# george-tyler-315-incline/ggml-neon-opt

Measured on AMD Instinct MI355X. Metric: tg128 tok/s + Q4_K GEMV achieved-HBM-GB/s, TinyLlama-1.1B Q4_K_M @1 GPU, higher is better.
Workload: dtype q4_K/q6_K x q8_K (u4/u6*i8 dot4 -> i32, f32 combine); 1 GPU; tinyllama-1.1b Q4_K_M tg2221: full decode graph, token i at position i of a fresh f16 KV cache; parallelism=replicas x1, hipgraph=True

## Files before the change

ggml-neon-opt_amd/csrc/kq_api.hip:

```cpp
#include <algorithm>
#include <stdio.h>
#include <stdlib.h>
#include <string.h>

#include <atomic>
#include <mutex>
#include <string>
#include <vector>

#include <hip/hip_ext.h>

#include "kq_common.h"
#include "kq_internal.h"

namespace kq {

template <int NCOL, bool FUSEDQ, bool DEBUG, int TMASK>
__global__ void kq_gemv(const GemvArgs a);
__global__ void kq_quantize_q8K(const float *x, int64_t x_stride, uint8_t *y, int nb, int64_t nblocks);
template <int TMASK, bool FUSEDQ, int PRO>
__global__ void kq_rows(const RowsArgs a);
template <int TMASK, bool FUSEDQ, int PRO>
__global__ void kq_rows_dyn(const RowsArgs a);
template <bool AM>
__global__ void kq_quantize_q8L(const float *x, int64_t x_stride, uint8_t *y, int nb, int64_t nblocks);
template <int TYPE, int RT, int CW>
__global__ void kq_mmq(const MmqArgs a);
template <int RT, int CW>
__global__ void kq_mmq_mixed(const MmqArgs a);
__global__ void kq_stream_ceiling(const uint8_t *buf, int64_t per_wave, int waves_total, uint32_t *sink);
__global__ void kq_quantize_f16img(const float *x, int64_t x_stride, uint8_t *img, uint8_t *bs, int nb, int64_t nblocks);
template <int TYPE, int NW>
__global__ void kq_mmf(const MmfArgs a);
__global__ void kq_mmf_reduce(const float *slab, int n_split, int m_cols, int n_rows, int slab_rows, float *y,
                              int64_t y_col_stride, const float *res, int64_t res_col_stride);

namespace {

constexpr int kMaxDevices = 64;
std::mutex g_dev_mu;
std::atomic<int> g_dev_state[kMaxDevices];
int g_dev_cus[kMaxDevices] = {0};

int current_device() {
    int dev = 0;
    if (hipGetDevice(&dev) != hipSuccess || dev < 0 || dev >= kMaxDevices) return -1;
    return dev;
}

void probe_device(int dev) {
    int n = 0;
    if (hipGetDeviceCount(&n) != hipSuccess || n <= 0 || dev >= n) {
        g_dev_state[dev].store(-1);
        return;
    }
    hipDeviceProp_t prop;
    if (hipGetDeviceProperties(&prop, dev) != hipSuccess) {
        g_dev_state[dev].store(-1);
        return;
    }
    if (strncmp(prop.gcnArchName, "gfx950", 6) != 0) {
        fprintf(stderr, "ggml_mi355x: device %d is %s, this library is built for gfx950 only\n", dev,
                prop.gcnArchName);
        g_dev_state[dev].store(-1);
        return;
    }
    g_dev_cus[dev] = prop.multiProcessorCount > 0 ? prop.multiProcessorCount : 256;
    g_dev_state[dev].store(1, std::memory_order_release);
}

template <int NCOL, bool FUSEDQ, bool DEBUG>
gemv_fn pick_tm(int tmask) {
    switch (tmask) {
        case 1: return kq_gemv<NCOL, FUSEDQ, DEBUG, 1>;
        case 4: return kq_gemv<NCOL, FUSEDQ, DEBUG, 4>;
        default: return kq_gemv<NCOL, FUSEDQ, DEBUG, 7>;
    }
}

gemv_fn pick_gemv(int ncol, bool fusedq, bool debug, int tmask) {
    if (debug) return pick_tm<1, false, true>(tmask);
    if (fusedq) return pick_tm<1, true, false>(tmask);
    switch (ncol) {
        case 1: return pick_tm<1, false, false>(tmask);
        case 2: return pick_tm<2, false, false>(tmask);
        case 4: return pick_tm<4, false, false>(tmask);
        default: return pick_tm<8, false, false>(tmask);
    }
}

int type_bit(int type) { return type == Q4_K ? 1 : type == Q5_K ? 2 : type == Q6_K ? 4 : 0; }

constexpr size_t kMaxLds = 160 * 1024;
constexpr size_t kTargetLds = 80 * 1024;
constexpr int64_t kFusedQMaxNb = 32;
constexpr int64_t kRowsFusedMaxNb = ROWS_QPASS * 4 * ROWS_WAVES;
constexpr double kRowsSmallBytes = 5e6;
std::atomic<int> g_rows_waves{0};

struct KnobDef {
    const char *name;
    double def;
};
const KnobDef kKnobs[KNOB_COUNT] = {
    {"GEMV_DIAG", 0},  {"GEMV_RING", 0},     {"GEMV_PRE0", 1},       {"GEMV_PF", 0},
    {"GEMV_XMODE", 0}, {"GEMV_SMALL_MB", kRowsSmallBytes / 1e6},      {"GEMV_WPC", 0},
    {"GEMV_SMALL_WG", 0}, {"GEMV_FQMAX", (double)kRowsFusedMaxNb},   {"MMF_WAVES", 0},
    {"MMF_ORDER", 0},  {"ATTN_DIAG", 0},     {"LOOPBACK_NOCOPY", 0}, {"ATTN_OPROJ", 1},
    {"AO_NRB", 0},     {"GEMV_DYN", 8},    {"GEMV_DYN_P", 0},      {"GEMV_DYN_STEPS", 16},
};
std::atomic<double> g_knob[KNOB_COUNT];
std::atomic<bool> g_knob_set[KNOB_COUNT];
std::atomic<uint32_t> g_knob_gen{0};


uint64_t *g_stamps = nullptr;
int64_t g_stamps_cap = 0;

struct OccKey {
    int dev;
    const void *fn;
    size_t lds;
};
int resident_wgs(const void *fn, size_t lds) {
    static std::mutex mu;
    static std::vector<std::pair<OccKey, int>> cache;
    const int dev = current_device();
    std::lock_guard<std::mutex> lk(mu);
    for (auto &e : cache)
        if (e.first.dev == dev && e.first.fn == fn && e.first.lds == lds) return e.second;
    int n = 0;
    if (lds > 64 * 1024) hipFuncSetAttribute(fn, hipFuncAttributeMaxDynamicSharedMemorySize, (int)kMaxLds);
    if (hipOccupancyMaxActiveBlocksPerMultiprocessor(&n, fn, WG_THREADS, lds) != hipSuccess || n <= 0) n = 1;
    if (n > 8) n = 8;
    cache.push_back({{dev, fn, lds}, n});
    return n;
}

}

double knob(Knob k) { return g_knob_set[k].load(std::memory_order_relaxed) ? g_knob[k].load() : kKnobs[k].def; }
uint32_t knob_generation() { return g_knob_gen.load(); }

struct TimedLaunch {
    std::string kernel;
    double bytes;
    hipEvent_t start, stop;
};
std::mutex g_tmu;
bool g_timing = false;
std::vector<TimedLaunch> g_tlog;
std::vector<std::pair<hipEvent_t, hipEvent_t>> g_tpool;
size_t g_tpool_used = 0;

bool capturing(hipStream_t s) {
    hipStreamCaptureStatus st = hipStreamCaptureStatusNone;
    if (hipStreamIsCapturing(s, &st) != hipSuccess) return false;
    return st != hipStreamCaptureStatusNone;
}

bool timing_slot(hipStream_t s, hipEvent_t &a, hipEvent_t &b) {
    std::lock_guard<std::mutex> lk(g_tmu);
    if (!g_timing || capturing(s)) return false;
    if (g_tpool_used == g_tpool.size()) {
        hipEvent_t e0, e1;
        if (hipEventCreate(&e0) != hipSuccess) return false;
        if (hipEventCreate(&e1) != hipSuccess) {
            hipEventDestroy(e0);
            return false;
        }
        g_tpool.push_back({e0, e1});
    }
    a = g_tpool[g_tpool_used].first;
    b = g_tpool[g_tpool_used].second;
    ++g_tpool_used;
    return true;
// ... 200 lines not shown
            if (((uintptr_t)d[i].w & 3u) != 0) return MI355X_E_INVAL;
            if (d[i].row_stride != (size_t)(nb * bb)) return MI355X_E_UNSUPPORTED;
            if (d[i].type != Q6_K && ((uintptr_t)d[i].w & 15u)) return MI355X_E_UNSUPPORTED;
        }
        bytes_total += (double)d[i].n_rows * bb;
        tmask |= type_bit(d[i].type);
    }
    if (tmask != 1 && tmask != 2 && tmask != 4) tmask = 7;
    pl.tmask = tmask;
    pl.fusedq = fusedq;
    pl.fn = pick_rows(tmask, fusedq, ROWS_PRO_NONE);
    a.n_desc = n_desc;
    a.nb = (int)nb;
    for (int i = 0; i < n_desc; ++i) {
        a.type[i] = d[i].type;
        a.w[i] = (const uint8_t *)d[i].w;
        a.y[i] = d[i].y;
        a.n_rows[i] = (int)d[i].n_rows;
    }
    {
        a.pf = (int)knob(KNOB_GEMV_PF);
        a.xmode = (int)knob(KNOB_GEMV_XMODE) & 7;
        a.diag = (int)knob(KNOB_GEMV_DIAG);
        const int pre = (int)knob(KNOB_GEMV_PRE0);
        a.pre0 = pre < 0 ? 0 : pre > 3 ? 3 : pre;
    }
    a.stamps = g_stamps;
    a.stamps_cap = g_stamps_cap;
    const double small_bytes = knob(KNOB_GEMV_SMALL_MB) * 1e6;
    if (waves_per_cu <= 0) {
        const int fixed = g_rows_waves.load();
        const int want = fixed > 0 ? fixed : bytes_total * nb < small_bytes ? ROWS_WAVES_SMALL : ROWS_WAVES;
        waves_per_cu = !fusedq || nb <= ROWS_QPASS * 4 * want ? want : ROWS_WAVES;
    }
    if (waves_per_cu > ROWS_WAVES) return MI355X_E_INVAL;
    pl.nwv = waves_per_cu;
    const int wpc_env = (int)knob(KNOB_GEMV_WPC);
    if (wpc_env > 0 && wpc_env < waves_per_cu) waves_per_cu = wpc_env;
    const int small_wg_env = (int)knob(KNOB_GEMV_SMALL_WG);
    int64_t n_wg = num_cus();
    if (small_wg_env > 0 && bytes_total * nb < small_bytes && small_wg_env < n_wg) n_wg = small_wg_env;
    const int64_t cap = n_wg * waves_per_cu;
    int64_t wv[MI355X_MAX_FUSED] = {0, 0, 0, 0};
    int64_t waves = 0;
    for (int i = 0; i < n_desc; ++i) {
        if (d[i].n_rows == 0) continue;
        const double share = (double)d[i].n_rows * block_bytes(d[i].type) / bytes_total;
        int64_t w = (int64_t)(share * (double)cap);
        const int64_t min_rows = (ROWS_SB + nb - 1) / nb;
        const int64_t wmax = (d[i].n_rows + min_rows - 1) / min_rows;
        if (w > wmax) w = wmax;
        if (w < 1) w = 1;
        wv[i] = w;
        waves += w;
    }
    while (waves > cap) {
        int big = 0;
        for (int i = 1; i < n_desc; ++i)
            if (wv[i] > wv[big]) big = i;
        --wv[big];
        --waves;
    }
    int64_t rpw = 0;
    waves = 0;
    for (int i = 0; i < n_desc; ++i) {
        a.wave_prefix[i] = (int)waves;
        if (wv[i] > 0) {
            a.rbase[i] = (int)(d[i].n_rows / wv[i]);
            a.rrem[i] = (int)(d[i].n_rows % wv[i]);
            const int64_t r = a.rbase[i] + (a.rrem[i] ? 1 : 0);
            rpw = r > rpw ? r : rpw;
        }
        waves += wv[i];
    }
    for (int i = n_desc; i <= MI355X_MAX_FUSED; ++i) a.wave_prefix[i] = (int)waves;
    a.waves_total = (int)waves;
    a.prio_bytes = 0;
    for (int i = 0; i < n_desc; ++i)
        if (wv[i] > 0) {
            const int64_t b = (int64_t)(a.rbase[i] + (a.rrem[i] ? 1 : 0)) * nb * block_bytes(d[i].type);
            a.prio_bytes = b > a.prio_bytes ? b : a.prio_bytes;
        }
    if (rpw > 0x7fffffff / 64) return MI355X_E_UNSUPPORTED;
    a.rpw = (int)(rpw > 0 ? rpw : 1);
    int g16 = ROWS_SB;
    while (nb % g16) g16 >>= 1;
    const int u = ROWS_SB / g16;
    int bR_full = (int)(ROWS_RECS / nb) / u * u;
    if (bR_full < u) bR_full = u;
    a.bR = a.rpw <= bR_full ? a.rpw : bR_full;
    const RowsLayout L = rows_layout((int)nb, tmask, a.bR, a.rpw, pl.nwv);
    if ((size_t)L.total > kMaxLds) return MI355X_E_UNSUPPORTED;
    pl.lds = (size_t)L.total;
    const int64_t grid = waves < n_wg ? waves : n_wg;
    pl.grid = dim3((unsigned)(grid > 0 ? grid : 1), 1, 1);
    pl.dyn = false;
    const double dyn_min = knob(KNOB_GEMV_DYN);
    const bool force = g_impl.load() == MI355X_GEMV_DYN;
    bool same_rows = true;
    for (int i = 1; i < n_desc; ++i) same_rows = same_rows && d[i].n_rows == d[0].n_rows;
    if (tmask != 7 && same_rows && (force || dyn_min > 0)) {
        int ush = 0;
        while ((int64_t)(1 << ush) * nb < ROWS_SB) ++ush;
        const double steps_per_wave = (double)n_desc * d[0].n_rows * nb / ROWS_SB / n_wg / pl.nwv;
        if ((int64_t)(1 << ush) * nb == ROWS_SB && steps_per_wave >= 16) ++ush;
        const int U = 1 << ush;
        const int Tu = (int)((U * nb + ROWS_SB - 1) / ROWS_SB);
        const int D = rows_depth(tmask == 1 ? Q4_K : tmask == 2 ? Q5_K : Q6_K);
        const int64_t flat = (int64_t)n_desc * ((d[0].n_rows + n_wg - 1) / n_wg);
        const int64_t rows = (int64_t)n_desc * d[0].n_rows;
        int bRd = (int)(ROWS_RECS / nb) / U * U;
        if (bRd < U) bRd = U;
        const double per_wave = (double)rows / (double)n_wg / U / pl.nwv;
        const bool auto_ok = per_wave >= dyn_min && steps_per_wave >= knob(KNOB_GEMV_DYN_STEPS);
        const RowsDynLayout DL = rows_dyn_layout((int)nb, tmask, bRd, (int)flat, pl.nwv);
        if ((force || auto_ok) && rows > 0 && (size_t)DL.total <= kMaxLds && flat < 0x7fffffff / 64) {
            pl.dyn = true;
            a.dyn_u = U;
            a.dyn_ush = ush;
            a.rbase[0] = (int)(d[0].n_rows / n_wg);
            a.rrem[0] = (int)(d[0].n_rows % n_wg);
            a.dyn_p = (D + Tu - 1) / Tu;
            const int p_knob = (int)knob(KNOB_GEMV_DYN_P);
            if (p_knob > 0) a.dyn_p = p_knob;
            a.bR = bRd;
            a.rpw = (int)flat;
            pl.lds = (size_t)DL.total;
            pl.grid = dim3((unsigned)n_wg, 1, 1);
            pl.fn = pick_rows(tmask, fusedq, ROWS_PRO_NONE, true);
        }
    }
    return MI355X_OK;
}

std::string rows_name(const RowsPlan &pl) {
    return std::string(pl.dyn ? "kq::kq_rows_dyn<" : "kq::kq_rows<") + std::to_string(pl.tmask) + ", " + (pl.fusedq ? "true" : "false") + ", " +
           std::to_string(pl.a.pro) + ">";
}

double rows_bytes(const RowsArgs &a, bool fusedq) {
    double w = 0, y = 0;
    for (int i = 0; i < a.n_desc; ++i) {
        const double rows = (double)a.n_rows[i];
        w += rows * a.nb * block_bytes(a.type[i]);
        y += rows * 4.0;
    }
    return w + y + (fusedq ? (double)a.nb * QK * 4.0 : (double)a.nb * Q8L_STRIDE);
}

int launch_rows(const RowsPlan &pl, hipStream_t stream) {
    const RowsArgs &a = pl.a;
    if (a.waves_total == 0) return MI355X_OK;
    allow_lds((const void *)pl.fn, pl.lds);
    hipEvent_t e0, e1;
    if (timing_slot(stream, e0, e1)) {
        hipExtLaunchKernelGGL(pl.fn, pl.grid, dim3(pl.nwv * 64), (uint32_t)pl.lds, stream, e0, e1, 0, a);
        timing_log(rows_name(pl), rows_bytes(a, pl.fusedq), e0, e1);
    } else {
        hipLaunchKernelGGL(pl.fn, pl.grid, dim3(pl.nwv * 64), pl.lds, stream, a);
    }
    const hipError_t e = hipGetLastError();
    return e == hipSuccess ? MI355X_OK : (int)e;
}

int launch_quantize_q8L(const float *x, int64_t x_stride_floats, void *y, int64_t k, int64_t nrows,
                        hipStream_t stream, bool mmq) {
    const auto kern = mmq ? kq_quantize_q8L<true> : kq_quantize_q8L<false>;
    const int64_t nb = k / QK;
    const int64_t nblocks = nb * nrows;
    if (nblocks == 0) return MI355X_OK;
    const int64_t wgs = (nblocks + 15) / 16;
    hipEvent_t e0, e1;
    if (timing_slot(stream, e0, e1)) {
        hipExtLaunchKernelGGL(kern, dim3((unsigned)wgs), dim3(WG_THREADS), 0, stream, e0, e1, 0, x,
                              x_stride_floats, (uint8_t *)y, (int)nb, nblocks);
        timing_log("kq::kq_quantize_q8L", (double)nblocks * (QK * 4.0 + Q8L_STRIDE), e0, e1);
    } else {
        hipLaunchKernelGGL(kern, dim3((unsigned)wgs), dim3(WG_THREADS), 0, stream, x, x_stride_floats,
                           (uint8_t *)y, (int)nb, nblocks);
    }
    const hipError_t e = hipGetLastError();
    return e == hipSuccess ? MI355X_OK : (int)e;
}

constexpr int64_t kMmqMinCols = 16;

std::atomic<int> g_mmq_impl{MI355X_MMQ_AUTO};
int mmq_impl() { return g_mmq_impl.load(); }

struct MmqShape {
    int rt, cw;
};
MmqShape mmq_shape(int type, int64_t rows, int64_t M) {
    const int impl = mmq_impl();
    if (impl == MI355X_MMQ_TILE128) return {128, 1};
    if (impl == MI355X_MMQ_TILE128W) return {128, 2};
    if (impl == MI355X_MMQ_TILE64W) return {64, 2};
    if (impl == MI355X_MMQ_TILE64) return {64, 1};
    if (impl == MI355X_MMQ_TILE128X) return {128, type == Q6_K ? 2 : 4};
    if (impl == MI355X_MMQ_TILE192) return type == Q6_K ? MmqShape{128, 1} : MmqShape{192, 1};
    const int64_t rt128 = (rows + 127) / 128;
    const int64_t g128x128 = rt128 * ((M + 127) / 128), g128x64 = rt128 * ((M + 63) / 64);
    if (type != Q6_K && g128x128 >= 160 && g128x128 < 384 && g128x64 >= 512) return {128, 1};
    if (g128x128 >= 160) return {128, 2};
    if (type == Q6_K && ((rows + 63) / 64) * ((M + 127) / 128) >= 192) return {64, 2};
    if (type != Q6_K && rt128 * ((M + 63) / 64) >= 256) return {128, 1};
    return {64, 1};
}
const void *mmq_fn(int type, bool mixed, MmqShape sh) {
#define KQ_MMQ_PICK(RT, CW)                                                      \
    return mixed          ? (const void *)kq_mmq_mixed<RT, CW>                 \
         : type == Q5_K ? (const void *)kq_mmq<Q5_K, RT, CW>                   \
         : type == Q6_K ? (const void *)kq_mmq<Q6_K, RT, CW>                   \
                        : (const void *)kq_mmq<Q4_K, RT, CW>;
    if (sh.rt == 192 && !mixed && type != Q6_K)
        return type == Q5_K ? (const void *)kq_mmq<Q5_K, 192, 1> : (const void *)kq_mmq<Q4_K, 192, 1>;
    if (sh.rt == 128 && sh.cw == 4 && !mixed && type != Q6_K)
        return type == Q5_K ? (const void *)kq_mmq<Q5_K, 128, 4> : (const void *)kq_mmq<Q4_K, 128, 4>;
    if (sh.rt == 128 && sh.cw == 2) KQ_MMQ_PICK(128, 2)
    if (sh.rt == 64 && sh.cw == 2) KQ_MMQ_PICK(64, 2)
    if (sh.rt == 128) KQ_MMQ_PICK(128, 1)
    KQ_MMQ_PICK(64, 1)
#undef KQ_MMQ_PICK
}
size_t mmq_lds(int type, MmqShape sh) {
    return (size_t)mmq_nbuf(type, sh.rt, sh.cw) * (size_t)mmq_buf_bytes(type, sh.rt, sh.cw) + 16 + MMQ_PF_LDS;
}

int launch_mmq(int type, const void *w, int64_t K, int64_t N, size_t row_stride, const uint8_t *xq, int64_t M,
               float *y, int64_t y_col_stride, hipStream_t stream, const float *res, int64_t res_col_stride) {
    MmqArgs a;
    memset(&a, 0, sizeof(a));
    a.n_mat = 1;
    a.res = res;
    a.res_col_stride = res_col_stride;
    a.w = (const uint8_t *)w;
    a.row_stride = (int64_t)row_stride;
    a.n_rows = (int)N;
    a.xq = xq;
    a.nb = (int)(K / QK);
    a.xq_col_stride = (int64_t)a.nb * Q8L_STRIDE;
    a.m_cols = (int)M;
    a.y = y;
    a.y_col_stride = y_col_stride;
    const MmqShape sh = mmq_shape(type, N, M);
    const void *fn = mmq_fn(type, false, sh);
    const size_t lds = mmq_lds(type, sh);
    const int cols = mmq_cols(sh.cw);
    dim3 grid((unsigned)((M + cols - 1) / cols), (unsigned)((N + sh.rt - 1) / sh.rt), 1);
    dim3 block((unsigned)(64 * mmq_waves(sh.rt, sh.cw)));
    std::string name = std::string("kq::kq_mmq<") + std::to_string(type) + ">";
    allow_lds(fn, lds);
    hipEvent_t e0, e1;
    const bool timed = timing_slot(stream, e0, e1);
    void *args[] = {&a};
    hipError_t e;
    if (timed) {
        e = hipExtLaunchKernel(fn, grid, block, args, lds, stream, e0, e1, 0);
        timing_log(name, (double)N * a.nb * block_bytes(type) + (double)M * a.nb * Q8L_STRIDE + (double)M * N * 4.0,
                   e0, e1);
    } else {
        e = hipLaunchKernel(fn, grid, block, args, lds, stream);
    }
    if (e != hipSuccess) return (int)e;
    e = hipGetLastError();
    return e == hipSuccess ? MI355X_OK : (int)e;
}

std::atomic<int> g_prefill{MI355X_PREFILL_EXACT};
int prefill_precision() { return g_prefill.load(); }

int mmf_nw(int64_t K) {
    const int v = (int)knob(KNOB_MMF_WAVES);
    return v == 4 || v == 8 ? v : K >= 8192 ? 8 : 4;
}
struct MmfPlan {
    int nw, n_ct, n_rt, n_split, nbs;
};
MmfPlan mmf_plan_nw(int64_t N, int64_t M, int64_t nb, int nw) {
    MmfPlan p;
    p.nw = nw;
    p.n_ct = (int)((M + MMF_COLS - 1) / MMF_COLS);
    p.n_rt = (int)((N + 32 * nw - 1) / (32 * nw));
    int s = 1;
    while ((int64_t)p.n_ct * p.n_rt * s < 256 && nb >= 8 * s) s *= 2;
    p.nbs = (int)((nb + s - 1) / s);
    p.n_split = (int)((nb + p.nbs - 1) / p.nbs);
    return p;
}
size_t al256(size_t v) { return (v + 255) & ~(size_t)255; }
size_t mmf_workspace(int64_t N, int64_t M, int64_t nb) {
    size_t w = al256((size_t)M * nb * MMF_IMG) + al256((size_t)M * nb * MMF_BSB), slab = 0;
    for (int nw = 4; nw <= 8; nw += 4) {
        const MmfPlan p = mmf_plan_nw(N, M, nb, nw);
        const size_t sb = p.n_split > 1 ? al256((size_t)p.n_split * M * N * 4) : 0;
        slab = sb > slab ? sb : slab;
    }
    return w + slab;
}
bool mmf_prefers(int type, int64_t N, int64_t K) {
    return prefill_precision() == MI355X_PREFILL_F16_ALL || type != Q4_K || N * K >= ((int64_t)32 << 20);
}
bool mmf_applies(int type, const void *w, int64_t N, size_t row_stride, int64_t M, int64_t K) {
    if (prefill_precision() < MI355X_PREFILL_F16) return false;
    if (!rows_enabled() || M < kMmqMinCols || N <= 0) return false;
    if (type != Q4_K && type != Q5_K && type != Q6_K) return false;
    if (N >= (1ll << 31) || M >= (1ll << 31)) return false;
    if (!mmf_prefers(type, N, K)) return false;
    if (type == Q6_K) return true;
    return ((uintptr_t)w & 15u) == 0 && (row_stride & 15u) == 0;
}

// ... 717 lines not shown
```

ggml-neon-opt_amd/csrc/kq_common.h:

```cpp
#pragma once

#include <hip/hip_runtime.h>
#include <stdint.h>

#include "ggml_mi355x.h"

namespace kq {

constexpr int QK = 256;
constexpr int WAVE = 64;
constexpr int WG_THREADS = 256;
constexpr int WAVES_PER_WG = WG_THREADS / WAVE;
constexpr int LANES_PER_BLOCK = 8;
constexpr int BLOCKS_PER_STEP = WAVE / LANES_PER_BLOCK;
constexpr int ACT_QS_STRIDE = 272;
constexpr int MAX_NCOL = 8;

constexpr int Q4_K = MI355X_TYPE_Q4_K;
constexpr int Q5_K = MI355X_TYPE_Q5_K;
constexpr int Q6_K = MI355X_TYPE_Q6_K;

__host__ __device__ constexpr int block_bytes(int type) {
    return type == Q4_K ? 144 : type == Q5_K ? 176 : type == Q6_K ? 210 : 0;
}

struct GemvArgs {
    int n_desc;
    int nb;
    int R;
    int m_total;
    int tasks_total;
    int out_per_wg;
    int diag;
    int ring;
    int ring_override;
    int task_prefix[MI355X_MAX_FUSED + 1];
    int type[MI355X_MAX_FUSED];
    int n_rows[MI355X_MAX_FUSED];
    const uint8_t *w[MI355X_MAX_FUSED];
    int64_t row_stride[MI355X_MAX_FUSED];
    float *y[MI355X_MAX_FUSED];
    int64_t y_col_stride[MI355X_MAX_FUSED];
    const float *x;
    int64_t x_col_stride;
    const uint8_t *xq;
    int64_t xq_col_stride;
    int32_t *dbg;
    uint64_t *stamps;
    int64_t stamps_cap;
};

struct LdsLayout {
    int ring, act, act_per_wave, act_col, recs, outs, spw, total;
};

__host__ __device__ inline LdsLayout lds_layout(int ncol, int nb, int out_per_wg, bool fusedq, int slot, int D) {
    LdsLayout L;
    L.spw = (nb + WAVES_PER_WG - 1) / WAVES_PER_WG;
    L.ring = 0;
    L.act = WAVES_PER_WG * D * slot;
    L.act_col = (L.spw * 292 + 16 + 15) & ~15;
    L.act_per_wave = fusedq ? L.spw * 1024 : ncol * L.act_col;
    L.recs = L.act + WAVES_PER_WG * L.act_per_wave;
    L.outs = L.recs + 2 * (WAVES_PER_WG - 1) * ncol * 8 * L.spw * 16;
    L.total = L.outs + out_per_wg * 4;
    return L;
}

#ifndef KQ_ROWS_WAVES
#define KQ_ROWS_WAVES 12
#endif
constexpr int ROWS_WAVES = KQ_ROWS_WAVES;
#ifndef KQ_ROWS_WAVES_SMALL
#define KQ_ROWS_WAVES_SMALL 6
#endif
constexpr int ROWS_WAVES_SMALL = KQ_ROWS_WAVES_SMALL;
constexpr int ROWS_QPASS = 3;
#ifndef KQ_ROWS_PF
#define KQ_ROWS_PF 2
#endif
constexpr int ROWS_PF = KQ_ROWS_PF;

struct RowsArgs {
    int n_desc;
    int nb;
    int rpw;
    int waves_total;
    int pre0;
    int pf;
    int bR;
    int xmode;
    int diag;
    int wave_prefix[MI355X_MAX_FUSED + 1];
    int rbase[MI355X_MAX_FUSED];
    int rrem[MI355X_MAX_FUSED];
    int type[MI355X_MAX_FUSED];
    const uint8_t *w[MI355X_MAX_FUSED];
    float *y[MI355X_MAX_FUSED];
    const float *x;
    const uint8_t *xq;
    uint64_t *stamps;
    int64_t stamps_cap;
    int pro;
    float eps;
    const float *x2;
    const float *res[MI355X_MAX_FUSED];
    int n_rows[MI355X_MAX_FUSED];
    int epi, epi_n, epi_wave_off;
    float *epi_y;
    int64_t prio_bytes;
    int dyn_u, dyn_p, dyn_ush;
};
constexpr int ROWS_PRO_NONE = 0, ROWS_PRO_NORM = 1, ROWS_PRO_SWIGLU = 2;
constexpr int ROWS_X_ROT = 1, ROWS_X_BAR = 2, ROWS_X_PIPE = 4;

constexpr int ROWS_SB = 16;
#ifndef KQ_MMQ_PF
#define KQ_MMQ_PF 0
#endif
constexpr int MMQ_PF_LDS = KQ_MMQ_PF ? 1024 : 0;
constexpr int Q8L_STRIDE = 304;
#ifndef KQ_MMQ_NBUF
#define KQ_MMQ_NBUF 2
#endif
__host__ __device__ constexpr int mmq_cgroups(int cw) { return cw == 4 ? 1 : 2; }
__host__ __device__ constexpr int mmq_cols(int cw) { return 32 * cw * mmq_cgroups(cw); }
__host__ __device__ constexpr int mmq_waves(int rt, int cw) { return rt / 32 * mmq_cgroups(cw); }
#ifndef KQ_MMQ_Q6_STRIDE
#define KQ_MMQ_Q6_STRIDE 240
#endif
static_assert(KQ_MMQ_Q6_STRIDE % 16 == 0 && KQ_MMQ_Q6_STRIDE >= 224, "whole granules");
__host__ __device__ constexpr int mmq_buf_bytes(int type, int rt, int cw) {
    return mmq_cols(cw) * Q8L_STRIDE + rt * (type == Q6_K ? KQ_MMQ_Q6_STRIDE : block_bytes(type));
}
__host__ __device__ constexpr int mmq_nbuf(int type, int rt, int cw) {
    return KQ_MMQ_NBUF == 1 ? 1 : KQ_MMQ_NBUF >= 3 && ((rt == 128 && cw == 1) || (rt == 64 && cw == 2)) &&
                   3 * mmq_buf_bytes(type, rt, cw) + 16 + MMQ_PF_LDS <= 160 * 1024
               ? 3
               : 2;
}
constexpr int ROWS_RECS = 64;
__host__ __device__ constexpr int rows_gran(int type) { return block_bytes(type) + 1; }
__host__ __device__ constexpr int rows_slot(int type) { return 16 * rows_gran(type); }
__host__ __device__ constexpr int rows_ni(int type) { return (rows_gran(type) + 63) / 64; }
#ifndef KQ_ROWS_DQ4
#define KQ_ROWS_DQ4 3
#endif
#ifndef KQ_ROWS_DQ6
#define KQ_ROWS_DQ6 2
#endif
__host__ __device__ constexpr int rows_depth(int type) {
    return type == Q4_K ? KQ_ROWS_DQ4 : type == Q5_K ? 3 : KQ_ROWS_DQ6;
}
__host__ __device__ constexpr int rows_ring_bytes(int type) { return rows_depth(type) * rows_slot(type); }
__host__ __device__ constexpr int cmax(int a, int b) { return a > b ? a : b; }
__host__ __device__ constexpr int rows_ring(int tmask) {
    return 16 + cmax((tmask & 1) ? rows_ring_bytes(Q4_K) : 0,
                     cmax((tmask & 2) ? rows_ring_bytes(Q5_K) : 0, (tmask & 4) ? rows_ring_bytes(Q6_K) : 0));
}

struct RowsLayout {
    int act, ring, ring_stride, recs, recs_stride, outs, outs_stride, sums, total;
};
__host__ __device__ inline RowsLayout rows_layout(int nb, int tmask, int bR, int rpw, int nwv) {
    RowsLayout L;
    L.act = 0;
    L.ring = nb * Q8L_STRIDE;
    L.ring_stride = rows_ring(tmask);
    L.recs = L.ring + nwv * L.ring_stride;
    L.recs_stride = bR * nb * 16;
    L.outs = L.recs + nwv * L.recs_stride;
    L.outs_stride = (rpw * 4 + 15) & ~15;
    L.sums = L.outs + nwv * L.outs_stride;
    L.total = L.sums + nb * 8;
    return L;
}

struct RowsDynLayout {
    int act, ring, ring_stride, recs, recs_stride, outs, sums, cnt, total;
};
__host__ __device__ inline RowsDynLayout rows_dyn_layout(int nb, int tmask, int bR, int flat_rows, int nwv) {
    RowsDynLayout L;
    L.act = 0;
    L.ring = nb * Q8L_STRIDE;
    L.ring_stride = rows_ring(tmask);
    L.recs = L.ring + nwv * L.ring_stride;
    L.recs_stride = bR * nb * 16;
    L.outs = L.recs + nwv * L.recs_stride;
    L.sums = L.outs + ((flat_rows * 4 + 15) & ~15);
    L.cnt = L.sums + nb * 8;
    L.total = L.cnt + 16;
    return L;
}

struct AttnArgs {
    const float *q, *k, *v;
    const int32_t *pos;
    const float *rope_table;
    uint16_t *k_cache;
    uint16_t *v_cache;
    float *out;
    int n_ctx, n_head, n_head_kv, head_dim;
    float scale;
    int diag;
    int rope_row;
    int no_store;
    uint8_t *q8_out;
    int v_lds;
    int n_tok;
};

struct AttnOprojArgs {
    AttnArgs at;
    const uint8_t *w;
    int64_t row_stride;
    int n_rows, nsb, R, n_rb;
    int head_lds;
    const float *res;
    float *y;
    uint8_t *recs;
    uint32_t *cnt;
};

constexpr int LAYER_WAVES = 8;
constexpr int LAYER_SYNC_U32 = 32 * 33;
struct LayerArgs {
    int G;
    int E, F, nb_e, nb_f, nq, nkv;
    int type[7];
    const uint8_t *w[7];
    float *y[3];
    const float *x;
    const float *attn_norm, *ffn_norm;
    float eps;
    float *att, *x1, *h, *x2;
    AttnArgs at;
    int n_attn, hpw, attn_stride, head_lds;
    uint32_t *sync;
    int *err;
    uint32_t expect[4][8];
    int D, slot;
    int o_aux, act_bytes, o_sums, o_res, lds;
    const uint8_t *tab;
    int64_t tab_stride;
    uint64_t *stamps;
    int64_t stamps_cap;
};

struct MmqArgs {
    const uint8_t *w;
    int64_t row_stride;
    int n_rows;
    const uint8_t *xq;
    int64_t xq_col_stride;
    int m_cols;
    float *y;
    int64_t y_col_stride;
    int nb;
    const float *res;
    int64_t res_col_stride;
    int n_mat;
    int tile0[5];
    int mtype[4];
    int kv_kind[4], kv_cur;
// ... 46 lines not shown
```

ggml-neon-opt_amd/csrc/kq_internal.h:

```cpp
#pragma once

#include <string>

#include "kq_common.h"

namespace kq {

int device_ok();
bool timing_slot(hipStream_t s, hipEvent_t &a, hipEvent_t &b);
void timing_log(const std::string &kernel, double bytes, hipEvent_t a, hipEvent_t b);
int num_cus();
int choose_ncol(int64_t M, int nb);
typedef void (*gemv_fn)(const GemvArgs);
struct GemvPlan {
    GemvArgs a;
    dim3 grid;
    size_t lds;
    gemv_fn fn;
    int ncol, tmask;
    bool fusedq, debug;
};
int plan_gemv(const mi355x_gemv_desc *d, int n_desc, int64_t K, int64_t M, int ncol, bool fusedq, bool debug,
              GemvPlan &pl);
int launch_gemv(const GemvPlan &pl, hipStream_t stream);
typedef void (*rows_fn)(const RowsArgs);
struct RowsPlan {
    RowsArgs a;
    dim3 grid;
    size_t lds;
    rows_fn fn;
    int tmask;
    bool fusedq;
    int nwv;
    bool dyn = false;
};
int plan_rows(const mi355x_gemv_desc *d, int n_desc, int64_t K, bool fusedq, RowsPlan &pl,
              int waves_per_cu = 0);
int launch_rows(const RowsPlan &pl, hipStream_t stream);
bool rows_enabled();
int launch_quantize(const float *x, int64_t x_stride_floats, void *y, int64_t k, int64_t nrows,
                    hipStream_t stream);
int gemv_m1(const mi355x_gemv_desc *d, int n, const float *x, int64_t k, void *ws, size_t ws_size,
            hipStream_t stream, const mi355x_gemv_ext *ext = nullptr);
int launch_rms_norm(const float *x, const float *w, float *y, int64_t n, int64_t nrows, float eps, hipStream_t s);
int launch_binary(int op, const float *a, const float *b, float *y, int64_t n, hipStream_t s,
                  int64_t nb = 0);
int launch_attn_prompt(const AttnArgs &a, int n_tok, hipStream_t s);
int attn_cells_reserve(const AttnArgs &a, hipStream_t stream);
bool attn_prompt_q8_ok(const AttnArgs &a);
bool mmq_applies(int type, const void *w, int64_t N, size_t row_stride, int64_t M);
int launch_quantize_q8L(const float *x, int64_t x_stride_floats, void *y, int64_t k, int64_t nrows,
                        hipStream_t stream, bool mmq = false);
int launch_mmq(int type, const void *w, int64_t K, int64_t N, size_t row_stride, const uint8_t *xq, int64_t M,
               float *y, int64_t y_col_stride, hipStream_t stream, const float *res = nullptr,
               int64_t res_col_stride = 0);
bool mmq_tile64(int type, int64_t N, int64_t M);
bool mmf_on();
bool mmf_applies(int type, const void *w, int64_t N, size_t row_stride, int64_t M, int64_t K);
bool mmf_prefers(int type, int64_t N, int64_t K);
int launch_f16img(const float *x, int64_t x_stride_floats, uint8_t *ws, int64_t K, int64_t M, hipStream_t stream);
int launch_mmf_gemm(int type, const void *w, int64_t K, int64_t N, size_t row_stride, uint8_t *ws, int64_t M,
                    float *y, int64_t y_col_stride, hipStream_t stream, const float *res = nullptr,
                    int64_t res_col_stride = 0);
int launch_mmf_multi(int type, int n_mat, const void *const *w, const int64_t *N, const size_t *row_stride,
                     float *const *y, const int64_t *y_col_stride, int64_t K, uint8_t *ws, size_t ws_size, int64_t M,
                     hipStream_t stream, const float *res = nullptr, int64_t res_col_stride = 0);
struct MmqKv {
    int kind[4];
    const int32_t *pos;
    const float *rope;
    uint16_t *k_cache, *v_cache;
    int n_ctx, hd;
};
int launch_mmq_multi(const int *types, int n_mat, const void *const *w, const int64_t *N, const size_t *row_stride,
                     float *const *y, const int64_t *y_col_stride, int64_t K, const uint8_t *xq, int64_t M,
                     hipStream_t stream, const MmqKv *kv = nullptr);
int launch_rms_norm_q8L(const float *x, const float *w, void *yq, int64_t n, int64_t nrows, float eps, hipStream_t s);
int launch_swiglu_q8L(const float *g, const float *u, void *yq, int64_t n, int64_t nrows, hipStream_t s);
int launch_swiglu(const float *g, const float *u, float *y, int64_t n, hipStream_t s);
int attn_args_from(const mi355x_attn_desc *d, AttnArgs &a);
int launch_attn(const AttnArgs &a, hipStream_t s);
bool attn_group_ok(const AttnArgs &a, int nwaves);
size_t attn_group_bytes(const AttnArgs &a, int nwaves);
constexpr size_t kAttnOprojCounterBytes = 1024;
constexpr int kAttnOprojMaxCtx = 256;
size_t attn_oproj_buffer(int hd, int n_head, int n_head_kv, int n_ctx, int type, int64_t K, int64_t n_rows, int *nsb);
int launch_attn_oproj(const AttnArgs &a, int type, const void *w, int64_t n_rows, size_t row_stride, const float *res,
                      float *y, uint8_t *buf, size_t buf_size, hipStream_t stream);
int attn_impl();
size_t attn_lds16(int hd, int n_ctx);
int layer_plan(LayerArgs &a, int hd, int n_head);
int launch_layer(const LayerArgs &a, hipStream_t stream);
int64_t layer_table_stride(const LayerArgs &a);
void layer_table_fill(const LayerArgs &a, uint8_t *buf, int64_t stride);
uint64_t *diag_stamps(int64_t *cap);
void allow_lds(const void *fn, size_t lds);
enum Knob {
    KNOB_GEMV_DIAG,
    KNOB_GEMV_RING,
    KNOB_GEMV_PRE0,
    KNOB_GEMV_PF,
    KNOB_GEMV_XMODE,
    KNOB_GEMV_SMALL_MB,
    KNOB_GEMV_WPC,
    KNOB_GEMV_SMALL_WG,
    KNOB_GEMV_FQMAX,
    KNOB_MMF_WAVES,
    KNOB_MMF_ORDER,
    KNOB_ATTN_DIAG,
    KNOB_LOOPBACK_NOCOPY,
    KNOB_ATTN_OPROJ,
    KNOB_AO_NRB,
    KNOB_GEMV_DYN,
    KNOB_GEMV_DYN_P,
    KNOB_GEMV_DYN_STEPS,
    KNOB_COUNT
};
double knob(Knob k);
uint32_t knob_generation();
uint64_t api_selector_key();
uint64_t ops_selector_key();

}
```

ggml-neon-opt_amd/csrc/kq_ops.hip:

```cpp
#include <math.h>
#include <stdlib.h>
#include <string.h>

#include <atomic>
#include <mutex>
#include <vector>

#include <hip/hip_ext.h>

#include "kq_common.h"
#include "kq_internal.h"
#include "kq_attn_device.h"
#include "kq_attn_head.h"
#include "kq_device.h"
#include "kq_ops_device.h"
#include "kq_rows_device.h"

#ifndef KQ_ATTN_BATCH_CTX
#define KQ_ATTN_BATCH_CTX 256
#endif
#ifndef KQ_ATTN_OSC1
#define KQ_ATTN_OSC1 0
#endif

namespace kq {

__global__ void __launch_bounds__(256) kq_get_rows(int type, const uint8_t *__restrict__ table, int64_t k,
                                                   int64_t row_stride, int64_t n_rows,
                                                   const int32_t *__restrict__ ids, float *__restrict__ out) {
    const int64_t r = blockIdx.y;
    const int64_t e0 = ((int64_t)blockIdx.x * 256 + threadIdx.x) * 8;
    if (e0 >= k) return;
    const int64_t id = ids[r];
    float *y = out + r * k + e0;
    if (id < 0 || id >= n_rows) {
#pragma unroll
        for (int i = 0; i < 8; ++i) y[i] = __builtin_nanf("");
        return;
    }
    const uint8_t *row = table + id * row_stride;
    if (type == MI355X_TYPE_F32) {
        const float *s = (const float *)row + e0;
#pragma unroll
        for (int i = 0; i < 8; ++i) y[i] = s[i];
        return;
    }
    const int64_t b = e0 / QK;
    const int e = (int)(e0 % QK);
    if (type == MI355X_TYPE_Q4_K || type == MI355X_TYPE_Q5_K) {
        const bool q5 = type == MI355X_TYPE_Q5_K;
        const uint8_t *blk = row + b * (q5 ? 176 : 144);
        const float d = h2f(*(const uint16_t *)blk), dmin = h2f(*(const uint16_t *)(blk + 2));
        const uint8_t *sc = blk + 4;
        const int j = e / 64, h = (e / 32) & 1, l0 = e % 32;
        const int is = 2 * j + h;
        int s, m;
        if (is < 4) {
            s = sc[is] & 63;
            m = sc[is + 4] & 63;
        } else {
            s = (sc[is + 4] & 0xF) | ((sc[is - 4] >> 6) << 4);
            m = (sc[is + 4] >> 4) | ((sc[is] >> 6) << 4);
        }
        const float d1 = d * (float)s, m1 = dmin * (float)m;
        const uint8_t *q = blk + (q5 ? 48 : 16) + 32 * j + l0;
        const uint8_t *qh = blk + 16 + l0;
#pragma unroll
        for (int i = 0; i < 8; ++i) {
            const int hb = q5 ? ((qh[i] >> (2 * j + h)) & 1) << 4 : 0;
            y[i] = __builtin_fmaf(d1, (float)(((q[i] >> (4 * h)) & 0xF) + hb), -m1);
        }
    } else {
        const uint8_t *blk = row + b * 210;
        const float d = h2f((uint16_t)(blk[208] | (blk[209] << 8)));
        const int half = e / 128, rr = e % 128, quarter = rr / 32, l0 = rr % 32;
        const uint8_t *ql = blk + 64 * half, *qh = blk + 128 + 32 * half;
        const int8_t *sc = (const int8_t *)(blk + 192) + 8 * half;
#pragma unroll
        for (int i = 0; i < 8; ++i) {
            const int l = l0 + i;
            int q;
            if (quarter == 0) q = (ql[l] & 0xF) | (((qh[l] >> 0) & 3) << 4);
            else if (quarter == 1) q = (ql[l + 32] & 0xF) | (((qh[l] >> 2) & 3) << 4);
            else if (quarter == 2) q = (ql[l] >> 4) | (((qh[l] >> 4) & 3) << 4);
            else q = (ql[l + 32] >> 4) | (((qh[l] >> 6) & 3) << 4);
            y[i] = d * (float)sc[l / 16 + 2 * quarter] * (float)(q - 32);
        }
    }
}

__global__ void __launch_bounds__(256) kq_rms_norm(const float *__restrict__ x, const float *__restrict__ w,
                                                   float *__restrict__ y, int64_t n, float eps) {
    extern __shared__ __attribute__((aligned(16))) double sb_sum[];
    const int64_t row = blockIdx.x;
    const float *xr = x + row * n;
    float *yr = y + row * n;
    const int nb = (int)(n / QK);
    const int rid = threadIdx.x >> 4, l = threadIdx.x & 15;
    for (int b0 = 0; b0 < nb; b0 += 16) {
        const int b = b0 + rid;
        double s = 0.0;
        if (b < nb) {
            float v[16];
            const float4 *p = (const float4 *)(xr + (int64_t)b * QK + 16 * l);
#pragma unroll
            for (int k = 0; k < 4; ++k) {
                const float4 t = p[k];
                v[4 * k] = t.x, v[4 * k + 1] = t.y, v[4 * k + 2] = t.z, v[4 * k + 3] = t.w;
            }
            s = sumsq16(v);
        }
        s = row16_sum(s);
        if (b < nb && l == 0) sb_sum[b] = s;
    }
    __syncthreads();
    double total = seq_sum_lds(sb_sum, nb);
    if (rms_mean_ambiguous(div_by_count(total, n), n)) {
        __syncthreads();
        if (threadIdx.x < 64) {
            const double s = seq_sumsq_wave(xr, n, threadIdx.x);
            if (threadIdx.x == 0) sb_sum[0] = s;
        }
        __syncthreads();
        total = sb_sum[0];
    }
    const float mean = (float)div_by_count(total, n);
    const float scale = 1.0f / sqrtf(mean + eps);
    for (int64_t i = threadIdx.x; i < n; i += 256) {
        const float v = xr[i] * scale;
        yr[i] = w ? v * w[i] : v;
    }
}

__global__ void __launch_bounds__(256) kq_binary(int op, const float *__restrict__ a, const float *__restrict__ b,
                                                 float *__restrict__ y, int64_t n, int64_t nb) {
    for (int64_t i = (int64_t)blockIdx.x * 256 + threadIdx.x; i < n; i += (int64_t)gridDim.x * 256) {
        const float bv = b[nb == n ? i : i % nb];
        y[i] = op == 0 ? a[i] + bv : a[i] * bv;
    }
}

__global__ void __launch_bounds__(256) kq_swiglu(const float *__restrict__ g, const float *__restrict__ u,
                                                 float *__restrict__ y, int64_t n) {
    const int64_t n4 = n & ~(int64_t)3;
    for (int64_t i = (int64_t)blockIdx.x * 256 + threadIdx.x; i < n; i += (int64_t)gridDim.x * 256)
        y[i] = i < n4 ? v_silu(g[i]) * u[i] : (g[i] / (1.0f + expf(-g[i]))) * u[i];
}

__global__ void __launch_bounds__(256) kq_rope(const float *__restrict__ x, float *__restrict__ y, int head_dim,
                                               int n_dims, int n_heads, const int32_t *__restrict__ pos_p,
                                               const float *__restrict__ table, int n_pos) {
    const int pos = *pos_p;
    const int per = head_dim / 2;
    const int64_t i = (int64_t)blockIdx.x * 256 + threadIdx.x;
    if (i >= (int64_t)n_heads * per) return;
    const int h = (int)(i / per), p = (int)(i % per);
    const float *s = x + (int64_t)h * head_dim + 2 * p;
    float *d = y + (int64_t)h * head_dim + 2 * p;
    if (pos < 0 || pos >= n_pos) {
        d[0] = d[1] = __builtin_nanf("");
        return;
    }
    if (2 * p >= n_dims) {
        d[0] = s[0];
        d[1] = s[1];
        return;
    }
    const float *cs = table + ((int64_t)pos * (n_dims / 2) + p) * 2;
    const float2 r = rope_pair(s[0], s[1], cs[0], cs[1]);
    d[0] = r.x;
    d[1] = r.y;
}

#ifndef KQ_ATTN_TPH64
#define KQ_ATTN_TPH64 256
#endif
#ifndef KQ_ATTN_KDMA1
#define KQ_ATTN_KDMA1 0
#endif
template <int HD, bool BATCH, int DS = 1, int TPH = 256, bool KD1 = false>
__global__ void __launch_bounds__(TPH) kq_attn_decode(const AttnArgs a) {
    extern __shared__ __attribute__((aligned(16))) uint8_t smem[];
    int h = blockIdx.x / DS, ds = blockIdx.x % DS;
    if ((a.n_head & 7) == 0) {
        const int x = blockIdx.x & 7, i = blockIdx.x >> 3;
        h = x * (a.n_head >> 3) + i / DS;
        ds = i % DS;
    }
    attn_head<HD, TPH, 0, KQ_ATTN_OSC1 != 0, false, BATCH, DS, KD1>(a, h, threadIdx.x, smem, a.out + (int64_t)h * HD,
                                                                     true, ds);
}

constexpr int ATTN_CHUNK = 64;
#ifndef KQ_ATTN_CELLS_OVER_SPLIT
#define KQ_ATTN_CELLS_OVER_SPLIT 0
#endif
#ifndef KQ_ATTN_CELLS_SLICES
#define KQ_ATTN_CELLS_SLICES 8
#endif
#ifndef KQ_ATTN_CELLS_MIN
#define KQ_ATTN_CELLS_MIN 1024
#endif
#ifndef KQ_ATTN_CELLS_OVERLAP
#define KQ_ATTN_CELLS_OVERLAP 1
#endif
#ifndef KQ_ATTN_CELLS_RS64
#define KQ_ATTN_CELLS_RS64 8
#endif
#ifndef KQ_ATTN_CELLS_RS128
#define KQ_ATTN_CELLS_RS128 16
#endif
#ifndef KQ_ATTN_CELLS_STOP
#define KQ_ATTN_CELLS_STOP 0
#endif
#ifndef KQ_ATTN_CELLS_VPAD
#define KQ_ATTN_CELLS_VPAD 64
#endif
constexpr int ATTN_CELLS_VPAD = KQ_ATTN_CELLS_VPAD;
constexpr int ATTN_CELLS_GMAX = 8;

template <int HD>
__global__ void __launch_bounds__(256) kq_attn_cells(const AttnArgs a, float *scores) {
    extern __shared__ __attribute__((aligned(16))) uint8_t smem[];
    constexpr int KV4 = HD / 8;
    constexpr int KPT = ATTN_CHUNK * KV4 / 256;
    const int g = blockIdx.y, c0 = blockIdx.x * ATTN_CHUNK, t = threadIdx.x;
    const int gsz = a.n_head / a.n_head_kv;
    const int kvw = a.n_head_kv * HD;
    uint4 kr[KPT];
#pragma unroll
    for (int u = 0; u < KPT; ++u) {
        const int i = t + 256 * u, r = i / KV4, k = i % KV4;
        kr[u] = *(const uint4 *)(a.k_cache + (int64_t)(c0 + r) * kvw + (int64_t)g * HD + 8 * k);
    }
    const int pos_in = *a.pos;
    const bool bad = pos_in < 0 || pos_in >= a.n_ctx;
    const int pos = bad ? 0 : pos_in;
    int n_kv = (pos + 1 + 31) / 32 * 32;
    n_kv = n_kv < a.n_ctx ? n_kv : a.n_ctx;
    if (c0 >= n_kv) return;
    uint16_t *q16 = (uint16_t *)smem;
    uint16_t *k16 = q16 + gsz * HD;
    uint4 *krow = (uint4 *)(k16 + HD);
    const bool holds = pos >= c0 && pos < c0 + ATTN_CHUNK;
#pragma unroll
    for (int u = 0; u < KPT; ++u) {
        const int i = t + 256 * u, r = i / KV4, k = i % KV4;
        krow[r * KV4 + (k ^ (r % KV4))] = kr[u];
    }
    const float *tc = a.rope_table + (a.rope_row ? 0 : (int64_t)pos * (HD / 2) * 2);
    for (int i = t; i < gsz * (HD / 2); i += 256) {
        const int hh = i / (HD / 2), p2 = i % (HD / 2);
        const float *qp = a.q + (int64_t)(g * gsz + hh) * HD + 2 * p2;
        const float2 rq = rope_pair(qp[0], qp[1], tc[2 * p2], tc[2 * p2 + 1]);
        q16[hh * HD + 2 * p2] = h2u(f2h_rne(rq.x));
        q16[hh * HD + 2 * p2 + 1] = h2u(f2h_rne(rq.y));
    }
    if (holds) {
        for (int p2 = t; p2 < HD / 2; p2 += 256) {
            const float *kp = a.k + (int64_t)g * HD + 2 * p2;
            const float2 rk = rope_pair(kp[0], kp[1], tc[2 * p2], tc[2 * p2 + 1]);
            const uint16_t k0 = h2u(f2h_rne(rk.x)), k1 = h2u(f2h_rne(rk.y));
            k16[2 * p2] = k0;
            k16[2 * p2 + 1] = k1;
            if (!bad) *(uint32_t *)(a.k_cache + (int64_t)pos * kvw + (int64_t)g * HD + 2 * p2) = k0 | ((uint32_t)k1 << 16);
        }
        for (int d = t; d < HD && !bad; d += 256)
            a.v_cache[(int64_t)(g * HD + d) * a.n_ctx + pos] = h2u(f2h_rne(a.v[(int64_t)g * HD + d]));
    }
    __syncthreads();
    for (int i = t; i < ATTN_CHUNK * gsz; i += 256) {
        const int r = i % ATTN_CHUNK, hh = i / ATTN_CHUNK, c = c0 + r;
        if (c >= n_kv) continue;
        float sc = -INFINITY;
        if (c <= pos) {
            uint4 kv[KV4];
            if (c == pos) {
#pragma unroll
                for (int k = 0; k < KV4; ++k) kv[k] = ((const uint4 *)k16)[k];
            } else {
#pragma unroll
                for (int k = 0; k < KV4; ++k) kv[k] = krow[r * KV4 + (k ^ (r % KV4))];
            }
            sc = vec_dot_f16_rows<HD>(kv, (const uint4 *)(q16 + hh * HD)) * a.scale;
        }
        scores[(int64_t)(g * gsz + hh) * a.n_ctx + c] = sc;
    }
}

template <int VM>
__device__ __forceinline__ void waitcnt_vm_le() {
    static_assert(VM >= 0 && VM < 64, "vmcnt is 6 bits");
    __builtin_amdgcn_s_waitcnt((VM & 15) | ((VM >> 4) << 14) | 0x0F70);
}
__device__ __forceinline__ void waitcnt_vm_floor8(int n) {
    switch ((n > 63 ? 63 : n) >> 3) {
    case 0: waitcnt_vm_le<0>(); break;
    case 1: waitcnt_vm_le<8>(); break;
    case 2: waitcnt_vm_le<16>(); break;
    case 3: waitcnt_vm_le<24>(); break;
    case 4: waitcnt_vm_le<32>(); break;
    case 5: waitcnt_vm_le<40>(); break;
    case 6: waitcnt_vm_le<48>(); break;
    default: waitcnt_vm_le<56>(); break;
    }
}
template <int HD, int DS>
__global__ void __launch_bounds__(256) kq_attn_cells_kqv(const AttnArgs a, const float *scores) {
    extern __shared__ __attribute__((aligned(16))) uint8_t smem[];
    constexpr int RS = HD / DS;
    static_assert(RS * 16 <= 256 && (RS & (RS - 1)) == 0 && RS >= 4, "16 threads per output, whole rows per wave");
    int h = blockIdx.x / DS, ds = blockIdx.x % DS;
    if ((a.n_head & 7) == 0) {
        const int x = blockIdx.x & 7, i = blockIdx.x >> 3;
        h = x * (a.n_head >> 3) + i / DS;
        ds = i % DS;
    }
    const int t = threadIdx.x, ln = t & 63;
    const int wv = __builtin_amdgcn_readfirstlane(t >> 6);
    const int g = h / (a.n_head / a.n_head_kv);
    const int pos_in = *a.pos;
    const bool bad = pos_in < 0 || pos_in >= a.n_ctx;
    const int pos = bad ? 0 : pos_in;
    int n_kv = (pos + 1 + 31) / 32 * 32;
    n_kv = n_kv < a.n_ctx ? n_kv : a.n_ctx;
    const int n_it = (pos + 32) / 32;
    float *w = (float *)smem;
    double *gsum = (double *)smem;
    uint16_t *p16 = (uint16_t *)smem;
    uint32_t *red = (uint32_t *)(w + a.n_ctx);
    float *scal = (float *)(red + RS * 16);
    uint8_t *vlds = (uint8_t *)(scal + 24);
    const int VSTR = 2 * a.n_ctx + ATTN_CELLS_VPAD;
    int nv = 0;
    {
// ... 520 lines not shown
    return check_launch();
}

int elem_grid(int64_t n) {
    int64_t g = (n + 255) / 256;
    return (int)(g < 4096 ? (g > 0 ? g : 1) : 4096);
}

int launch_rms_norm(const float *x, const float *w, float *y, int64_t n, int64_t nrows, float eps, hipStream_t s) {
    if (nrows == 0) return MI355X_OK;
    return timed_launch("kq::kq_rms_norm", (double)nrows * n * 8 + (w ? n * 4.0 : 0.0), kq_rms_norm,
                        dim3((unsigned)nrows), dim3(256), (size_t)(n / QK) * 8 + 8, s, x, w, y, n, eps);
}

int launch_binary(int op, const float *a, const float *b, float *y, int64_t n, hipStream_t s, int64_t nb) {
    if (n == 0) return MI355X_OK;
    if (nb <= 0) nb = n;
    if (n % nb) return MI355X_E_INVAL;
    return timed_launch(op == 0 ? "kq::kq_add" : "kq::kq_mul", n * 8.0 + nb * 4.0, kq_binary, dim3(elem_grid(n)),
                        dim3(256), 0, s, op, a, b, y, n, nb);
}

int launch_swiglu(const float *g, const float *u, float *y, int64_t n, hipStream_t s) {
    if (n == 0) return MI355X_OK;
    return timed_launch("kq::kq_swiglu", n * 12.0, kq_swiglu, dim3(elem_grid(n)), dim3(256), 0, s, g, u, y, n);
}

int attn_group_waves(const AttnArgs &a) {
    const int gsz = a.n_head / a.n_head_kv;
    return gsz < 4 ? 4 : gsz > 16 ? 16 : gsz;
}

size_t attn_group_bytes(const AttnArgs &a, int nwaves) {
    const int gsz = a.n_head / a.n_head_kv;
    return (size_t)attn_group_lds(a.head_dim, a.n_ctx, gsz < nwaves ? gsz : nwaves).total;
}

bool attn_group_ok(const AttnArgs &a, int nwaves) {
    const uintptr_t m = (uintptr_t)a.q | (uintptr_t)a.k | (uintptr_t)a.v;
    return (m & 7u) == 0 && a.diag == 0 && attn_group_bytes(a, nwaves) <= 160 * 1024;
}

#ifndef KQ_ATTN_DEFAULT_IMPL
#define KQ_ATTN_DEFAULT_IMPL MI355X_ATTN_SPLIT
#endif
std::atomic<int> g_attn_impl{KQ_ATTN_DEFAULT_IMPL};
int attn_impl() { return g_attn_impl.load(); }

size_t attn_cells_lds_a(int hd, int gsz) { return (size_t)gsz * hd * 2 + (size_t)hd * 2 + (size_t)ATTN_CHUNK * hd * 2; }
size_t attn_cells_lds_b(int n_ctx, int rs) {
    return (size_t)n_ctx * 4 + (size_t)rs * 64 + 96 + (size_t)rs * (2 * (size_t)n_ctx + ATTN_CELLS_VPAD);
}
int attn_cells_rs(int hd, int n_ctx) {
    if (hd == 64) return KQ_ATTN_CELLS_RS64;
    return attn_cells_lds_b(n_ctx, KQ_ATTN_CELLS_RS128) <= 160 * 1024 ? KQ_ATTN_CELLS_RS128 : 8;
}

struct CellsScratch {
    struct Entry {
        int dev;
        hipStream_t stream;
        void *p;
        size_t bytes;
    };
    std::mutex mu;
    std::vector<Entry> cur;
};
CellsScratch &cells_scratch() {
    static CellsScratch s;
    return s;
}
void *attn_cells_buffer(size_t bytes, hipStream_t stream, bool may_alloc) {
    int dev = 0;
    if (hipGetDevice(&dev) != hipSuccess) return nullptr;
    CellsScratch &cs = cells_scratch();
    std::lock_guard<std::mutex> lk(cs.mu);
    for (auto &e : cs.cur)
        if (e.dev == dev && e.stream == stream) {
            if (e.bytes >= bytes) return e.p;
            if (!may_alloc) return nullptr;
            void *p = nullptr;
            if (hipMalloc(&p, bytes) != hipSuccess) return nullptr;
            e.p = p, e.bytes = bytes;
            return p;
        }
    if (!may_alloc) return nullptr;
    void *p = nullptr;
    if (hipMalloc(&p, bytes) != hipSuccess) return nullptr;
    cs.cur.push_back({dev, stream, p, bytes});
    return p;
}

bool attn_cells_applies(const AttnArgs &a) {
    const int gsz = a.n_head_kv > 0 ? a.n_head / a.n_head_kv : 0;
    return attn_impl() == MI355X_ATTN_SPLIT && a.n_ctx > KQ_ATTN_CELLS_MIN && a.n_ctx % ATTN_CHUNK == 0 &&
           a.n_ctx <= 1024 * ATTN_CELLS_GMAX &&
           (a.head_dim == 64 || a.head_dim == 128) && gsz >= 1 && gsz <= 16 &&
           (KQ_ATTN_CELLS_OVER_SPLIT || attn_slices(a) == 1 || attn_slices(a) >= KQ_ATTN_CELLS_SLICES) &&
           attn_cells_lds_b(a.n_ctx, attn_cells_rs(a.head_dim, a.n_ctx)) <= 160 * 1024 && ((uintptr_t)a.k_cache & 15u) == 0 &&
           ((uintptr_t)a.v_cache & 15u) == 0;
}

int attn_cells_reserve(const AttnArgs &a, hipStream_t stream) {
    if (!attn_cells_applies(a)) return MI355X_OK;
    return attn_cells_buffer((size_t)a.n_head * a.n_ctx * 4, stream, true) ? MI355X_OK : MI355X_E_WORKSPACE;
}

template <int HD, int RS>
int launch_attn_cells_t(const AttnArgs &a, float *ws, hipStream_t s, const char *na, const char *nb) {
    const int gsz = a.n_head / a.n_head_kv;
    const size_t la = attn_cells_lds_a(HD, gsz), lb = attn_cells_lds_b(a.n_ctx, RS);
    const dim3 ga((unsigned)(a.n_ctx / ATTN_CHUNK), (unsigned)a.n_head_kv);
    const int rc = timed_launch(na, 0.0, kq_attn_cells<HD>, ga, dim3(256), la, s, a, ws);
    if (rc) return rc;
    allow_lds((const void *)kq_attn_cells_kqv<HD, HD / RS>, lb);
    return timed_launch(nb, 0.0, kq_attn_cells_kqv<HD, HD / RS>, dim3((unsigned)(a.n_head * (HD / RS))), dim3(256), lb, s,
                        a, (const float *)ws);
}
int launch_attn_cells(const AttnArgs &a, float *ws, hipStream_t s) {
    if (a.head_dim == 64)
        return launch_attn_cells_t<64, KQ_ATTN_CELLS_RS64>(a, ws, s, "kq::kq_attn_cells<64>", "kq::kq_attn_cells_kqv<64>");
    if (attn_cells_rs(128, a.n_ctx) == KQ_ATTN_CELLS_RS128)
        return launch_attn_cells_t<128, KQ_ATTN_CELLS_RS128>(a, ws, s, "kq::kq_attn_cells<128>", "kq::kq_attn_cells_kqv<128>");
    return launch_attn_cells_t<128, 8>(a, ws, s, "kq::kq_attn_cells<128>", "kq::kq_attn_cells_kqv<128>");
}

int attn_path(const AttnArgs &a) {
    if (attn_impl() == MI355X_ATTN_GROUP && attn_group_ok(a, attn_group_waves(a))) return MI355X_ATTN_PATH_GROUP;
    const int ds = attn_slices(a);
    if (ds > 1 && !attn_cells_applies(a)) return ds == 4 ? MI355X_ATTN_PATH_SPLIT4 : MI355X_ATTN_PATH_SPLIT8;
    if (attn_cells_applies(a)) return MI355X_ATTN_PATH_CELLS;
    if (KQ_ATTN_KDMA1 && a.n_ctx <= KQ_ATTN_BATCH_CTX && a.n_ctx % 8 == 0 && ((uintptr_t)a.v_cache & 15u) == 0 &&
        ((uintptr_t)a.k_cache & 15u) == 0)
        return MI355X_ATTN_PATH_KD1;
    return a.n_ctx > KQ_ATTN_BATCH_CTX ? MI355X_ATTN_PATH_HEAD_BATCH : MI355X_ATTN_PATH_HEAD;
}

int launch_attn(const AttnArgs &a, hipStream_t s) {
    const double bytes = 0;
    const int path = attn_path(a);
    if (path == MI355X_ATTN_PATH_GROUP) {
        const int nw = attn_group_waves(a);
        const size_t glds = attn_group_bytes(a, nw);
        if (a.head_dim == 64) {
            allow_lds((const void *)kq_attn_group<64>, glds);
            return timed_launch("kq::kq_attn_group<64>", bytes, kq_attn_group<64>, dim3(a.n_head_kv), dim3(64 * nw),
                                glds, s, a);
        }
        allow_lds((const void *)kq_attn_group<128>, glds);
        return timed_launch("kq::kq_attn_group<128>", bytes, kq_attn_group<128>, dim3(a.n_head_kv), dim3(64 * nw),
                            glds, s, a);
    }
    AttnArgs b = a;
    const int ds = attn_slices(a);
    if (path == MI355X_ATTN_PATH_SPLIT4 || path == MI355X_ATTN_PATH_SPLIT8) {
        const size_t lds = attn_lds_v(a.head_dim, a.n_ctx, ds);
        const dim3 grid((unsigned)(a.n_head * ds));
#define KQ_ATTN_SPLIT_LAUNCH(HD, DS)                                                                        \
    if (a.head_dim == HD && ds == DS) {                                                                    \
        allow_lds((const void *)kq_attn_decode<HD, true, DS>, lds);                                        \
        return timed_launch("kq::kq_attn_decode<" #HD ", true, " #DS ">", bytes, kq_attn_decode<HD, true, DS>, \
                            grid, dim3(256), lds, s, b);                                                   \
    }
        KQ_ATTN_SPLIT_LAUNCH(64, 4)
        KQ_ATTN_SPLIT_LAUNCH(64, 8)
        KQ_ATTN_SPLIT_LAUNCH(128, 4)
        KQ_ATTN_SPLIT_LAUNCH(128, 8)
#undef KQ_ATTN_SPLIT_LAUNCH
        return MI355X_E_INVAL;
    }
    if (path == MI355X_ATTN_PATH_CELLS) {
        hipStreamCaptureStatus cst = hipStreamCaptureStatusNone;
        const bool capturing = hipStreamIsCapturing(s, &cst) == hipSuccess && cst != hipStreamCaptureStatusNone;
        void *ws = attn_cells_buffer((size_t)a.n_head * a.n_ctx * 4, s, !capturing);
        if (ws) return launch_attn_cells(a, (float *)ws, s);
    }
    if (path == MI355X_ATTN_PATH_KD1) {
        const size_t lds = attn_lds_v(a.head_dim, a.n_ctx, 1, true);
        if (a.head_dim == 64) {
            allow_lds((const void *)kq_attn_decode<64, true, 1, 256, true>, lds);
            return timed_launch("kq::kq_attn_decode<64, true, 1, kd1>", bytes, kq_attn_decode<64, true, 1, 256, true>,
                                dim3(a.n_head), dim3(256), lds, s, b);
        }
        allow_lds((const void *)kq_attn_decode<128, true, 1, 256, true>, lds);
        return timed_launch("kq::kq_attn_decode<128, true, 1, kd1>", bytes, kq_attn_decode<128, true, 1, 256, true>,
                            dim3(a.n_head), dim3(256), lds, s, b);
    }
    b.v_lds = a.n_ctx > KQ_ATTN_BATCH_CTX && a.n_ctx % 8 == 0 && attn_lds_v(a.head_dim, a.n_ctx) <= 160 * 1024 &&
              ((uintptr_t)a.v_cache & 15u) == 0 && KQ_ATTN_VLDS;
    const size_t lds = b.v_lds ? attn_lds_v(a.head_dim, a.n_ctx) : attn_lds(a.head_dim, a.n_ctx);
    const bool batch = a.n_ctx > KQ_ATTN_BATCH_CTX;
    if (a.head_dim == 64) {
        if (!batch)
            return timed_launch("kq::kq_attn_decode<64, false>", bytes, kq_attn_decode<64, false, 1, KQ_ATTN_TPH64>,
                                dim3(a.n_head), dim3(KQ_ATTN_TPH64), lds, s, b);
        if (b.v_lds) allow_lds((const void *)kq_attn_decode<64, true>, lds);
        return timed_launch("kq::kq_attn_decode<64, true>", bytes, kq_attn_decode<64, true>, dim3(a.n_head), dim3(256), lds, s, b);
    }
    if (!batch) return timed_launch("kq::kq_attn_decode<128, false>", bytes, kq_attn_decode<128, false>, dim3(a.n_head), dim3(256), lds, s, b);
    if (b.v_lds) allow_lds((const void *)kq_attn_decode<128, true>, lds);
    return timed_launch("kq::kq_attn_decode<128, true>", bytes, kq_attn_decode<128, true>, dim3(a.n_head), dim3(256), lds, s, b);
}

std::atomic<int> g_prompt_impl{MI355X_ATTN_GROUP};

bool attn_prompt_group_ok(const AttnArgs &a) {
    const int gsz = a.n_head / a.n_head_kv;
    return gsz <= PROMPT_GMAX && attn_prompt_group_lds(a.head_dim, a.n_ctx, gsz) <= 160 * 1024 &&
           g_prompt_impl.load() == MI355X_ATTN_GROUP;
}
int attn_prompt_tpw(const AttnArgs &a) {
    const int gsz = a.n_head / a.n_head_kv;
    return KQ_PROMPT_TPW > 1 && (gsz == 4 || gsz == 8) &&
                   attn_prompt_group_lds(a.head_dim, a.n_ctx, gsz * KQ_PROMPT_TPW) <= 160 * 1024
               ? KQ_PROMPT_TPW
               : 1;
}

bool attn_prompt_q8_ok(const AttnArgs &a) {
    return attn_prompt_group_ok(a) && ((a.n_head / a.n_head_kv) * a.head_dim) % QK == 0 &&
           a.n_ctx >= a.head_dim;
}

int launch_attn_prompt(const AttnArgs &a0, int n_tok, hipStream_t s) {
    if (n_tok <= 0) return MI355X_OK;
    AttnArgs a = a0;
    a.n_tok = n_tok;
    const size_t lds = attn_prompt_lds(a.head_dim, a.n_ctx);
    const int gsz = a.n_head / a.n_head_kv;
    const bool group = attn_prompt_group_ok(a);
    if (a.q8_out && !group) return MI355X_E_INVAL;
    const int tpw = group ? attn_prompt_tpw(a) : 1;
    const size_t glds = attn_prompt_group_lds(a.head_dim, a.n_ctx, gsz * tpw);
    const dim3 gs((unsigned)n_tok, (unsigned)a.n_head_kv), ga((unsigned)a.n_head, (unsigned)n_tok);
    const dim3 gg((unsigned)a.n_head_kv, (unsigned)((n_tok + tpw - 1) / tpw));
    int rc;
#define KQ_PROMPT_GROUP_LAUNCH(HD, G, T)                                                                  \
    {                                                                                                   \
        allow_lds((const void *)kq_attn_prompt_group<HD, G, T>, glds);                                  \
        return timed_launch("kq::kq_attn_prompt_group<" #HD ">", 0.0, kq_attn_prompt_group<HD, G, T>, gg, \
                            dim3(256), glds, s, a);                                                     \
    }
    if (a.head_dim == 64) {
        rc = a.no_store ? 0 : timed_launch("kq::kq_kv_store<64>", 0.0, kq_kv_store<64>, gs, dim3(256), 0, s, a);
        if (rc) return rc;
        if (group) {
            if (gsz == 8 && tpw > 1) KQ_PROMPT_GROUP_LAUNCH(64, 8, KQ_PROMPT_TPW)
            if (gsz == 4 && tpw > 1) KQ_PROMPT_GROUP_LAUNCH(64, 4, KQ_PROMPT_TPW)
            if (gsz == 8) KQ_PROMPT_GROUP_LAUNCH(64, 8, 1)
            if (gsz == 4) KQ_PROMPT_GROUP_LAUNCH(64, 4, 1)
            KQ_PROMPT_GROUP_LAUNCH(64, 0, 1)
        }
        allow_lds((const void *)kq_attn_prompt<64>, lds);
        return timed_launch("kq::kq_attn_prompt<64>", 0.0, kq_attn_prompt<64>, ga, dim3(256), lds, s, a);
    }
    rc = a.no_store ? 0 : timed_launch("kq::kq_kv_store<128>", 0.0, kq_kv_store<128>, gs, dim3(256), 0, s, a);
    if (rc) return rc;
    if (group) {
        if (gsz == 8 && tpw > 1) KQ_PROMPT_GROUP_LAUNCH(128, 8, KQ_PROMPT_TPW)
        if (gsz == 4 && tpw > 1) KQ_PROMPT_GROUP_LAUNCH(128, 4, KQ_PROMPT_TPW)
        if (gsz == 8) KQ_PROMPT_GROUP_LAUNCH(128, 8, 1)
        if (gsz == 4) KQ_PROMPT_GROUP_LAUNCH(128, 4, 1)
        KQ_PROMPT_GROUP_LAUNCH(128, 0, 1)
    }
#undef KQ_PROMPT_GROUP_LAUNCH
    allow_lds((const void *)kq_attn_prompt<128>, lds);
    return timed_launch("kq::kq_attn_prompt<128>", 0.0, kq_attn_prompt<128>, ga, dim3(256), lds, s, a);
}

int check_attn(const AttnArgs &a) {
    if (!a.q || !a.k || !a.v || !a.pos || !a.rope_table || !a.k_cache || !a.v_cache || !a.out) return MI355X_E_INVAL;
    if (a.head_dim != 64 && a.head_dim != 128) return MI355X_E_UNSUPPORTED;
    if (a.n_head <= 0 || a.n_head_kv <= 0 || a.n_head % a.n_head_kv) return MI355X_E_INVAL;
    if (a.n_ctx < 32 || a.n_ctx % 32 || a.n_ctx > 8192) return MI355X_E_UNSUPPORTED;
    if (((uintptr_t)a.k_cache & 15u) || ((uintptr_t)a.v_cache & 15u)) return MI355X_E_INVAL;
    if (attn_lds(a.head_dim, a.n_ctx) > 64 * 1024) return MI355X_E_UNSUPPORTED;
    return MI355X_OK;
}

uint64_t ops_selector_key() {
    return (uint64_t)(uint32_t)attn_impl() | ((uint64_t)(uint32_t)g_prompt_impl.load() << 8);
}

}

using namespace kq;

extern "C" {

int mi355x_get_rows(int type, const void *table, int64_t ne0, size_t row_stride, int64_t n_rows, const int32_t *ids,
                    int64_t n_ids, float *dst, void *stream) {
    if (!table || !ids || !dst || ne0 <= 0 || n_ids < 0 || n_rows < 0) return MI355X_E_INVAL;
    if (type != MI355X_TYPE_F32 && type != MI355X_TYPE_Q4_K && type != MI355X_TYPE_Q5_K && type != MI355X_TYPE_Q6_K)
        return MI355X_E_UNSUPPORTED;
    if (ne0 % (type == MI355X_TYPE_F32 ? 8 : QK)) return MI355X_E_INVAL;
    if (row_stride < mi355x_row_size(type, ne0) && type != MI355X_TYPE_F32) return MI355X_E_INVAL;
    if (n_ids == 0) return MI355X_OK;
    if (!device_ok()) return MI355X_E_NODEVICE;
    const dim3 grid((unsigned)((ne0 / 8 + 255) / 256), (unsigned)n_ids);
    return timed_launch("kq::kq_get_rows", (double)n_ids * (ne0 * 4.0 + (double)mi355x_row_size(type, ne0)),
                        kq_get_rows, grid, dim3(256), 0, (hipStream_t)stream, type, (const uint8_t *)table, ne0,
                        (int64_t)row_stride, n_rows, ids, dst);
}

int mi355x_rms_norm(const float *x, const float *w, float *y, int64_t n, int64_t nrows, float eps, void *stream) {
    if (!x || !y || n <= 0 || nrows < 0 || !(eps >= 0.0f)) return MI355X_E_INVAL;
    if (n % QK || ((uintptr_t)x & 15u)) return MI355X_E_UNSUPPORTED;
    if (!device_ok()) return MI355X_E_NODEVICE;
    return launch_rms_norm(x, w, y, n, nrows, eps, (hipStream_t)stream);
}

int mi355x_add(const float *a, const float *b, float *y, int64_t n, void *stream) {
    if (!a || !b || !y || n < 0) return MI355X_E_INVAL;
    if (!device_ok()) return MI355X_E_NODEVICE;
    return launch_binary(0, a, b, y, n, (hipStream_t)stream);
}

int mi355x_mul(const float *a, const float *b, float *y, int64_t n, void *stream) {
    if (!a || !b || !y || n < 0) return MI355X_E_INVAL;
    if (!device_ok()) return MI355X_E_NODEVICE;
    return launch_binary(1, a, b, y, n, (hipStream_t)stream);
}

int mi355x_swiglu(const float *gate, const float *up, float *y, int64_t n, void *stream) {
    if (!gate || !up || !y || n < 0) return MI355X_E_INVAL;
    if (!device_ok()) return MI355X_E_NODEVICE;
    return launch_swiglu(gate, up, y, n, (hipStream_t)stream);
}

size_t mi355x_rope_table_size(int n_pos, int n_dims) {
    if (n_pos <= 0 || n_dims <= 0 || n_dims % 2) return 0;
    return (size_t)n_pos * (size_t)(n_dims / 2) * 2 * sizeof(float);
}

int mi355x_rope_table(float *table, int n_pos, int n_dims, float freq_base, float freq_scale, void *stream) {
    const size_t bytes = mi355x_rope_table_size(n_pos, n_dims);
    if (!table || !bytes || !(freq_base > 0.0f)) return MI355X_E_INVAL;
    if (!device_ok()) return MI355X_E_NODEVICE;
    std::vector<float> host(bytes / sizeof(float));
    const float theta_scale = powf(freq_base, -2.0f / (float)n_dims);
    for (int p = 0; p < n_pos; ++p) {
        float theta = (float)p;
        for (int i = 0; i < n_dims / 2; ++i) {
            const float th = freq_scale * theta;
            host[((size_t)p * (n_dims / 2) + i) * 2 + 0] = cosf(th) * 1.0f;
            host[((size_t)p * (n_dims / 2) + i) * 2 + 1] = sinf(th) * 1.0f;
            theta *= theta_scale;
        }
    }
    hipError_t e = hipMemcpyAsync(table, host.data(), bytes, hipMemcpyHostToDevice, (hipStream_t)stream);
    if (e == hipSuccess) e = hipStreamSynchronize((hipStream_t)stream);
    return e == hipSuccess ? MI355X_OK : (int)e;
}

int mi355x_rope(const float *x, float *y, int head_dim, int n_dims, int n_heads, const int32_t *pos,
// ... 79 lines not shown
```

ggml-neon-opt_amd/csrc/kq_rows.hip:

```cpp
#include <hip/hip_ext.h>

#include "kq_internal.h"
#include "kq_ops_device.h"
#include "kq_rows_device.h"

#ifndef KQ_ROWS_DIAG
#define KQ_ROWS_DIAG 0
#endif
#if KQ_ROWS_DIAG
#define RDIAG(a) ((a).diag)
#define RSTAMPS(a) ((a).stamps)
#else
#define RDIAG(a) 0
#define RSTAMPS(a) ((uint64_t *)nullptr)
#endif

#ifndef KQ_ROWS_XMODE
#define KQ_ROWS_XMODE 0
#endif
#ifndef KQ_ROWS_PRE0
#define KQ_ROWS_PRE0 1
#endif
#ifndef KQ_ROWS_L2PF
#define KQ_ROWS_L2PF 0
#endif
#ifndef KQ_ROWS_MASKED
#define KQ_ROWS_MASKED 2
#endif
#ifndef KQ_ROWS_LINT_BREAK
#define KQ_ROWS_LINT_BREAK 0
#endif

#ifndef KQ_ROWS_PRIO
#define KQ_ROWS_PRIO 0
#endif

#ifndef KQ_ROWS_YSC1
#define KQ_ROWS_YSC1 1
#endif

namespace kq {

__device__ __forceinline__ void store_y(float *p, float v) {
    if (KQ_ROWS_YSC1) asm volatile("global_store_dword %0, %1, off sc1" ::"v"(p), "v"(v) : "memory");
    else *p = v;
}

template <bool AM>
__global__ void __launch_bounds__(WG_THREADS) kq_quantize_q8L(const float *__restrict__ x, int64_t x_stride,
                                                              uint8_t *__restrict__ y, int nb, int64_t nblocks) {
    const int lane = threadIdx.x & 63;
    const int64_t bi = (int64_t)blockIdx.x * 16 + (threadIdx.x >> 4);
    if (bi >= nblocks) return;
    const int64_t row = bi / nb;
    const int b = (int)(bi - row * nb);
    const float *xb = x + row * x_stride + (int64_t)b * QK + 16 * (lane & 15);
    u32x4 v[4];
#pragma unroll
    for (int k = 0; k < 4; ++k) v[k] = *(const u32x4 *)(xb + 4 * k);
    quant16_store<AM>(v, lane & 15, y + bi * Q8L_STRIDE);
}
template __global__ void kq_quantize_q8L<false>(const float *, int64_t, uint8_t *, int, int64_t);
template __global__ void kq_quantize_q8L<true>(const float *, int64_t, uint8_t *, int, int64_t);

__global__ void __launch_bounds__(256) kq_rms_norm_q8L(const float *__restrict__ x, const float *__restrict__ w,
                                                       uint8_t *__restrict__ yq, int64_t n, float eps) {
    extern __shared__ __attribute__((aligned(16))) double sb_sum[];
    const int64_t row = blockIdx.x;
    const float *xr = x + row * n;
    const int nb = (int)(n / QK);
    const int rid = threadIdx.x >> 4, l = threadIdx.x & 15;
    for (int b0 = 0; b0 < nb; b0 += 16) {
        const int b = b0 + rid;
        double s = 0.0;
        if (b < nb) {
            float v[16];
            const float4 *p = (const float4 *)(xr + (int64_t)b * QK + 16 * l);
#pragma unroll
            for (int k = 0; k < 4; ++k) {
                const float4 t = p[k];
                v[4 * k] = t.x, v[4 * k + 1] = t.y, v[4 * k + 2] = t.z, v[4 * k + 3] = t.w;
            }
            s = sumsq16(v);
        }
        s = row16_sum(s);
        if (b < nb && l == 0) sb_sum[b] = s;
    }
    __syncthreads();
    double total = seq_sum_lds(sb_sum, nb);
    if (rms_mean_ambiguous(div_by_count(total, n), n)) {
        __syncthreads();
        if (threadIdx.x < 64) {
            const double s = seq_sumsq_wave(xr, n, threadIdx.x);
            if (threadIdx.x == 0) sb_sum[0] = s;
        }
        __syncthreads();
        total = sb_sum[0];
    }
    const float mean = (float)div_by_count(total, n);
    const float scale = 1.0f / sqrtf(mean + eps);
    for (int b0 = 0; b0 < nb; b0 += 16) {
        const int b = b0 + rid;
        if (b >= nb) continue;
        const float4 *p = (const float4 *)(xr + (int64_t)b * QK + 16 * l);
        const float4 *q = (const float4 *)(w + (int64_t)b * QK + 16 * l);
        u32x4 v[4];
#pragma unroll
        for (int k = 0; k < 4; ++k) {
            const float4 t = p[k], m = q[k];
            v[k].x = __float_as_uint((t.x * scale) * m.x);
            v[k].y = __float_as_uint((t.y * scale) * m.y);
            v[k].z = __float_as_uint((t.z * scale) * m.z);
            v[k].w = __float_as_uint((t.w * scale) * m.w);
        }
        quant16_store<true>(v, l, yq + (row * nb + b) * Q8L_STRIDE);
    }
}

__global__ void __launch_bounds__(256) kq_swiglu_q8L(const float *__restrict__ g, const float *__restrict__ u,
                                                     uint8_t *__restrict__ yq, int nb, int64_t nblocks) {
    const int64_t bi = (int64_t)blockIdx.x * 16 + (threadIdx.x >> 4);
    if (bi >= nblocks) return;
    const int l = threadIdx.x & 15;
    const int64_t e0 = bi * QK + 16 * l;
    u32x4 v[4];
#pragma unroll
    for (int k = 0; k < 4; ++k) {
        const float4 gv = *(const float4 *)(g + e0 + 4 * k), uv = *(const float4 *)(u + e0 + 4 * k);
        v[k].x = __float_as_uint(v_silu(gv.x) * uv.x);
        v[k].y = __float_as_uint(v_silu(gv.y) * uv.y);
        v[k].z = __float_as_uint(v_silu(gv.z) * uv.z);
        v[k].w = __float_as_uint(v_silu(gv.w) * uv.w);
    }
    (void)nb;
    quant16_store<true>(v, l, yq + bi * Q8L_STRIDE);
}

int launch_rms_norm_q8L(const float *x, const float *w, void *yq, int64_t n, int64_t nrows, float eps, hipStream_t s) {
    if (nrows == 0) return MI355X_OK;
    hipEvent_t e0, e1;
    const size_t lds = (size_t)(n / QK) * 8 + 8;
    if (timing_slot(s, e0, e1)) {
        hipExtLaunchKernelGGL(kq_rms_norm_q8L, dim3((unsigned)nrows), dim3(256), (uint32_t)lds, s, e0, e1, 0, x, w,
                              (uint8_t *)yq, n, eps);
        timing_log("kq::kq_rms_norm_q8L", (double)nrows * (n * 4.0 + (n / QK) * (double)Q8L_STRIDE) + n * 4.0, e0, e1);
    } else {
        hipLaunchKernelGGL(kq_rms_norm_q8L, dim3((unsigned)nrows), dim3(256), lds, s, x, w, (uint8_t *)yq, n, eps);
    }
    const hipError_t e = hipGetLastError();
    return e == hipSuccess ? MI355X_OK : (int)e;
}

int launch_swiglu_q8L(const float *g, const float *u, void *yq, int64_t n, int64_t nrows, hipStream_t s) {
    const int64_t nb = n / QK, nblocks = nb * nrows;
    if (nblocks == 0) return MI355X_OK;
    const int64_t wgs = (nblocks + 15) / 16;
    hipEvent_t e0, e1;
    if (timing_slot(s, e0, e1)) {
        hipExtLaunchKernelGGL(kq_swiglu_q8L, dim3((unsigned)wgs), dim3(256), 0, s, e0, e1, 0, g, u, (uint8_t *)yq,
                              (int)nb, nblocks);
        timing_log("kq::kq_swiglu_q8L", (double)nblocks * (QK * 8.0 + Q8L_STRIDE), e0, e1);
    } else {
        hipLaunchKernelGGL(kq_swiglu_q8L, dim3((unsigned)wgs), dim3(256), 0, s, g, u, (uint8_t *)yq, (int)nb, nblocks);
    }
    const hipError_t e = hipGetLastError();
    return e == hipSuccess ? MI355X_OK : (int)e;
}

template <int TYPE, bool FUSEDQ, int PRO>
__device__ __forceinline__ void rows_body(const RowsArgs &a, const WaveWork &ww, uint8_t *smem, const RowsLayout &L,
                                          int wave, int lane, uint64_t st0) {
    constexpr int BSZ = block_bytes(TYPE);
    constexpr int GRAN = rows_gran(TYPE);
    constexpr int NI = rows_ni(TYPE);
    constexpr int SLOT = rows_slot(TYPE);
    constexpr int D = rows_depth(TYPE);
    static_assert(D >= 2 && D <= 4, "vm_wait_k covers 3 steps in flight");
    const int nb = a.nb, bR = a.bR;
    const int nwv = __builtin_amdgcn_readfirstlane((int)(blockDim.x >> 6));
    const int q = lane >> 2, s = lane & 3;
    uint8_t *const ring = smem + L.ring + wave * L.ring_stride;
    uint8_t *const ring_end = ring + D * SLOT;
    Rec *const recs = (Rec *)(smem + L.recs + wave * L.recs_stride);
    float *const outs = (float *)(smem + L.outs + wave * L.outs_stride);
    const uint8_t *const actq = smem + L.act;

    const int G = ww.nrows * nb;
    const int T = (G + ROWS_SB - 1) / ROWS_SB;
    const uint8_t *src = a.w[ww.m] + (int64_t)ww.r0 * nb * BSZ;
    const uint32_t mis = (uint32_t)((uintptr_t)src & 15u);
    const uint8_t *s16 = src - mis;
    const uint8_t *last16 =
        G > 0 ? (const uint8_t *)((uintptr_t)(src + (int64_t)G * BSZ - 1) & ~(uintptr_t)15) : s16;

    const bool pf_on = FUSEDQ && (KQ_ROWS_L2PF < 0 ? a.pf != 0 : KQ_ROWS_L2PF != 0) && T > D + 1;
    uint32_t pf_sink = 0;
    uint8_t *islot = ring;
    int it_ = 0;
    auto issue = [&]() {
        const uint8_t *base = s16 + (int64_t)it_ * (ROWS_SB * BSZ) + 16 * lane;
        if (it_ + 1 < T) {
#pragma unroll
            for (int i = 0; i < NI; ++i)
                if (i + 1 < NI || lane < GRAN - 64 * (NI - 1)) dma16_nt(base + 1024 * i, (LDS void *)(islot + 1024 * i));
        } else {
#pragma unroll
            for (int i = 0; i < NI; ++i) {
                const uint8_t *p = base + 1024 * i;
                if (i + 1 < NI || lane < GRAN - 64 * (NI - 1))
                    dma16_nt(p < last16 ? p : last16, (LDS void *)(islot + 1024 * i));
            }
        }
        islot = islot + SLOT == ring_end ? ring : islot + SLOT;
        ++it_;
    };

    const float *const res_p = a.res[ww.m];
    uint32_t rv = 0;

    const int pre_req = KQ_ROWS_PRE0 < 0 ? a.pre0 : KQ_ROWS_PRE0;
    const int pre_cap = pre_req < D ? pre_req : D;
    const int pre0 = T >= pre_cap ? pre_cap : (T > 0 ? T : 0);
    uint64_t sx = 0, sq = 0, sf = 0;
    if (FUSEDQ) {
        const int PASS = 4 * nwv;
        const int xm = KQ_ROWS_XMODE >= 0 ? KQ_ROWS_XMODE : a.xmode;
        u32x4 xv[ROWS_QPASS][4] = {};
        u32x4 x2v[ROWS_QPASS][4] = {};
        const int qiters = (nb + PASS - 1) / PASS;
        int qw = 0;
#pragma unroll
        for (int i = 0; i < ROWS_QPASS; ++i) qw += (i < qiters && PASS * i + 4 * wave < nb) ? 1 : 0;
        const int rot = (xm & ROWS_X_ROT) ? (int)(blockIdx.x % (unsigned)nb) : 0;
        auto sbk = [&](int j) {
            int b = (j < nb ? j : nb - 1) + rot;
            return b >= nb ? b - nb : b;
        };
        constexpr int pro = PRO;
        constexpr int PL = PRO != ROWS_PRO_NONE ? 8 : 4;
#pragma unroll
        for (int i = 0; i < ROWS_QPASS; ++i) {
            if (i < qw) {
                const int b = sbk(PASS * i + 4 * wave + (lane >> 4));
                const float *xp = a.x + (int64_t)b * QK + 16 * (lane & 15);
#pragma unroll
                for (int k = 0; k < 4; ++k) xv[i][k] = gload16_asm(xp + 4 * k);
                if (PRO != ROWS_PRO_NONE) {
                    const float *x2p = ((RDIAG(a) & 16) ? a.x : a.x2) + (int64_t)b * QK + 16 * (lane & 15);
#pragma unroll
                    for (int k = 0; k < 4; ++k) x2v[i][k] = gload16_asm(x2p + 4 * k);
                }
            }
        }
        rv = gload4_asm(res_p && ww.nrows > 0 ? res_p + ww.r0 + (lane < ww.nrows ? lane : 0) : a.x);
        if (xm & ROWS_X_BAR) asm volatile("s_barrier" ::: "memory");
        constexpr bool kConstPre = KQ_ROWS_PRE0 == 1 && KQ_ROWS_L2PF == 0;
        if (kConstPre && T == 0) {
            const uint8_t *xb = (const uint8_t *)a.x + 16 * lane;
#pragma unroll
            for (int i = 0; i < NI; ++i)
                if (KQ_ROWS_MASKED && i + 1 == NI) dma16_nt_lanes(xb, (LDS void *)(islot + 1024 * i), lane, GRAN - 64 * (NI - 1));
                else if (i + 1 < NI || lane < GRAN - 64 * (NI - 1)) dma16_nt(xb, (LDS void *)(islot + 1024 * i));
        }
        if (KQ_ROWS_MASKED && kConstPre && T > 0) {
            const uint8_t *base = s16 + 16 * lane;
            const uint8_t *lim = T > 1 ? base + 1024 * (NI - 1) : base + 1024 * (NI - 1) < last16 ? base + 1024 * (NI - 1) : last16;
#pragma unroll
            for (int i = 0; i + 1 < NI; ++i) {
                const uint8_t *p = base + 1024 * i;
                dma16_nt(T > 1 || p < last16 ? p : last16, (LDS void *)(islot + 1024 * i));
            }
            dma16_nt_lanes(lim, (LDS void *)(islot + 1024 * (NI - 1)), lane, GRAN - 64 * (NI - 1));
            islot = islot + SLOT == ring_end ? ring : islot + SLOT;
            ++it_;
        } else {
            for (int j = 0; j < pre0; ++j) issue();
        }
        if (pf_on) {
            const uint8_t *p = s16 + (int64_t)D * (ROWS_SB * BSZ) + 64 * lane;
#pragma unroll
            for (int i = 0; i < ROWS_PF; ++i) l2_touch(p + 4096 * i < last16 ? p + 4096 * i : last16, pf_sink);
        }
        const int tail = 1 + NI * pre0 + (pf_on ? ROWS_PF : 0);
        auto pin = [&]() {
            asm volatile("" : "+v"(xv[0][0]), "+v"(xv[0][1]), "+v"(xv[0][2]), "+v"(xv[0][3]), "+v"(xv[1][0]),
                         "+v"(xv[1][1]), "+v"(xv[1][2]), "+v"(xv[1][3]), "+v"(xv[2][0]), "+v"(xv[2][1]),
                         "+v"(xv[2][2]), "+v"(xv[2][3]));
            if (pro != ROWS_PRO_NONE) {
#pragma unroll
                for (int i = 0; i < ROWS_QPASS; ++i)
#pragma unroll
                    for (int k = 0; k < 4; ++k) asm volatile("" : "+v"(x2v[i][k]));
            }
        };
        if (pro != ROWS_PRO_NORM && (xm & ROWS_X_PIPE)) {
#pragma unroll
            for (int i = 0; i < ROWS_QPASS; ++i) {
                if (i < qw) {
                    vm_wait_dyn((qw - 1 - i) * PL + tail);
                    pin();
                    if (pro == ROWS_PRO_SWIGLU && !(RDIAG(a) & 32)) {
#pragma unroll
                        for (int k = 0; k < 4; ++k) xv[i][k] = swiglu4(xv[i][k], x2v[i][k]);
                    }
                    const int j = PASS * i + 4 * wave + (lane >> 4);
                    if (j < nb && !(RDIAG(a) & 64)) quant16_store(xv[i], lane & 15, smem + L.act + Q8L_STRIDE * sbk(j));
                }
            }
            if (RSTAMPS(a)) sx = sq = __builtin_amdgcn_s_memrealtime();
        } else {
            if (KQ_ROWS_LINT_BREAK) {
            } else if (kConstPre && KQ_ROWS_MASKED == 2) {
                vm_wait<NI + 1>();
            } else if (kConstPre) {
                vm_wait<NI>();
            } else {
                vm_wait_dyn(tail);
            }
            pin();
            if (RDIAG(a) & 32) {
            } else if (pro == ROWS_PRO_SWIGLU) {
#pragma unroll
                for (int i = 0; i < ROWS_QPASS; ++i)
                    if (i < qw)
#pragma unroll
                        for (int k = 0; k < 4; ++k) xv[i][k] = swiglu4(xv[i][k], x2v[i][k]);
            } else if (pro == ROWS_PRO_NORM) {
                double *sums = (double *)(smem + L.sums);
#pragma unroll
                for (int i = 0; i < ROWS_QPASS; ++i) {
                    if (i < qw) {
                        const int j = PASS * i + 4 * wave + (lane >> 4);
                        double sq = 0.0;
                        if (j < nb) {
                            float v[16];
#pragma unroll
                            for (int k = 0; k < 4; ++k) {
                                v[4 * k] = __uint_as_float(xv[i][k].x), v[4 * k + 1] = __uint_as_float(xv[i][k].y);
                                v[4 * k + 2] = __uint_as_float(xv[i][k].z), v[4 * k + 3] = __uint_as_float(xv[i][k].w);
                            }
                            sq = sumsq16(v);
                        }
                        sq = row16_sum(sq);
                        if (j < nb && (lane & 15) == 0) sums[sbk(j)] = sq;
                    }
                }
                asm volatile("s_waitcnt lgkmcnt(0)\n\ts_barrier" ::: "memory");
                double tot = seq_sum_lanes(sums, nb, lane);
                if (rms_mean_ambiguous(div_by_count(tot, (int64_t)nb * QK), (int64_t)nb * QK))
                    tot = seq_sumsq_wave(a.x, (int64_t)nb * QK, lane);
                const float mean = (float)div_by_count(tot, (int64_t)nb * QK);
                const float scale = 1.0f / sqrtf(mean + a.eps);
#pragma unroll
                for (int i = 0; i < ROWS_QPASS; ++i)
                    if (i < qw)
#pragma unroll
                        for (int k = 0; k < 4; ++k) xv[i][k] = normmul4(xv[i][k], x2v[i][k], scale);
            }
            if (RSTAMPS(a)) sx = __builtin_amdgcn_s_memrealtime();
#pragma unroll 1
            for (int i = 0; i < qw; ++i) {
                u32x4 cur[4];
#pragma unroll
                for (int k = 0; k < 4; ++k) cur[k] = i == 0 ? xv[0][k] : i == 1 ? xv[1][k] : xv[2][k];
                const int j = PASS * i + 4 * wave + (lane >> 4);
                if (j < nb && !(RDIAG(a) & 64)) quant16_store(cur, lane & 15, smem + L.act + Q8L_STRIDE * sbk(j));
            }
            if (RSTAMPS(a)) {
                asm volatile("s_waitcnt lgkmcnt(0)" ::: "memory");
                sq = __builtin_amdgcn_s_memrealtime();
            }
        }
    } else {
        const int ng = nb * (Q8L_STRIDE / 16);
        for (int j = wave; 64 * j < ng; j += nwv) {
            const int k = 64 * j + lane;
            if (k < ng) dma16(a.xq + 16 * k, (LDS void *)(smem + L.act + 1024 * j));
        }
        for (int j = 0; j < pre0; ++j) issue();
        vm_wait_k<NI>(pre0);
    }
    while (it_ < D && it_ < T) issue();
    asm volatile("s_waitcnt lgkmcnt(0)\n\ts_barrier" ::: "memory");
    const uint64_t st1 = RSTAMPS(a) ? __builtin_amdgcn_s_memrealtime() : 0;

    int io = q, rr = 0;
    while (io >= nb) {
        io -= nb;
        ++rr;
    }
    int bend = bR * nb < G ? bR * nb : G;
    int brow = 0;
    const uint8_t *cslot = ring;
    int prio = -1;
#pragma unroll 1
    for (int t = 0; t < T; ++t) {
        if (KQ_ROWS_PRIO && (t & 3) == 0) {
            const int64_t rem = (int64_t)(T - t) * (ROWS_SB * BSZ);
            int p = (int)(rem * 4 / (a.prio_bytes + 1));
            p = __builtin_amdgcn_readfirstlane(p > 3 ? 3 : p);
            if (p != prio) {
                prio = p;
                if (p == 3) __builtin_amdgcn_s_setprio(3);
                else if (p == 2) __builtin_amdgcn_s_setprio(2);
                else if (p == 1) __builtin_amdgcn_s_setprio(1);
                else __builtin_amdgcn_s_setprio(0);
            }
        }
        if (pf_on && t < pre0) {
            if (T - t >= D) vm_wait<NI * (D - 1) + ROWS_PF>();
            else vm_wait_kp<NI, ROWS_PF>(T - t - 1);
        } else if (T - t >= D) {
            vm_wait<NI * (D - 1)>();
        } else {
            vm_wait_k<NI>(T - t - 1);
        }
        if (!(RDIAG(a) & 8) && ROWS_SB * t + q < G) {
            const uint8_t *blk = cslot + mis + q * BSZ;
            const uint8_t *ab = actq + io * Q8L_STRIDE;
            QuadOut r = TYPE == Q4_K ? quad_q4K(blk, ab, s) : TYPE == Q5_K ? quad_q5K(blk, ab, s) : quad_q6K(blk, ab, s);
            const int isum = quad_sum(r.isum);
            const int imin = quad_sum(r.imin);
            if (s == 0) {
                const float yd = *(const float *)ab;
                Rec rec;
                if (TYPE == Q6_K) {
                    rec.a = isum - 32 * imin;
                    rec.b = 0;
                    rec.c = h2f(r.dh) * yd;
                    rec.e = 0.f;
                } else {
                    rec.a = isum;
                    rec.b = imin;
                    rec.c = yd * h2f(r.dh & 0xffffu);
                    rec.e = yd * h2f(r.dh >> 16);
                }
                recs[io * bR + rr] = rec;
            }
        }
        cslot = cslot + SLOT == ring_end ? ring : cslot + SLOT;
        io += ROWS_SB;
        if (nb >= ROWS_SB) {
            if (io >= nb) {
                io -= nb;
                ++rr;
            }
        } else {
            while (io >= nb) {
                io -= nb;
                ++rr;
            }
        }
        if (it_ < T) issue();
        if (RSTAMPS(a) && t == 0) sf = __builtin_amdgcn_s_memrealtime();
        if (ROWS_SB * (t + 1) >= bend) {
            wave_lds_fence();
            const int nr = bR < ww.nrows - brow ? bR : ww.nrows - brow;
            if (lane < nr) {
                float v = 0.f;
                const Rec *rc = recs + lane;
#pragma unroll 4
                for (int i = 0; i < nb; ++i) v = chain_step(TYPE, rc[i * bR], v);
                outs[brow + lane] = v;
            }
            brow += bR;
            rr -= bR;
            bend = bend + bR * nb < G ? bend + bR * nb : G;
            wave_lds_fence();
        }
    }
    if (KQ_ROWS_PRIO) __builtin_amdgcn_s_setprio(0);
    const uint64_t st2 = RSTAMPS(a) ? __builtin_amdgcn_s_memrealtime() : 0;
    if (pf_on) {
        asm volatile("" ::"v"(pf_sink));
    }

    if (ww.nrows > 0) {
        wave_lds_fence();
        float *y = a.y[ww.m] + ww.r0;
        if (res_p) {
            asm volatile("s_waitcnt vmcnt(0)" ::: "memory");
            asm volatile("" : "+v"(rv));
            for (int k = 0; k < ww.nrows; k += 64)
                if (k + lane < ww.nrows)
                    store_y(y + k + lane, outs[k + lane] + (k == 0 ? __uint_as_float(rv) : res_p[ww.r0 + k + lane]));
        } else {
            for (int k = 0; k < ww.nrows; k += 64)
                if (k + lane < ww.nrows) store_y(y + k + lane, outs[k + lane]);
        }
    }
    if (a.epi && !(RDIAG(a) & 128)) {
        asm volatile("s_waitcnt lgkmcnt(0)\n\ts_barrier" ::: "memory");
        if (ww.m == 1 && ww.nrows > 0) {
            const float *gouts = (const float *)(smem + L.outs + (wave - a.epi_wave_off) * L.outs_stride);
            const int n4 = a.epi_n & ~3;
            for (int k = 0; k < ww.nrows; k += 64)
                if (k + lane < ww.nrows) {
                    const int r = ww.r0 + k + lane;
                    const float gv = gouts[k + lane], uv = outs[k + lane];
                    store_y(a.epi_y + r, r < n4 ? v_silu(gv) * uv : (gv / (1.0f + expf(-gv))) * uv);
                }
        }
    }
    if (RSTAMPS(a)) {
        const int64_t o = ((int64_t)blockIdx.x * ROWS_WAVES + wave) * 8;
        if (lane == 0 && o + 7 < a.stamps_cap) {
            RSTAMPS(a)[o] = st0;
            RSTAMPS(a)[o + 1] = st1;
            RSTAMPS(a)[o + 2] = st2;
            RSTAMPS(a)[o + 3] = __builtin_amdgcn_s_memrealtime();
            RSTAMPS(a)[o + 4] = sx;
            RSTAMPS(a)[o + 5] = sq;
            RSTAMPS(a)[o + 6] = sf;
        }
    }
}

template <int TMASK, bool FUSEDQ, int PRO>
__global__ void __launch_bounds__(ROWS_WAVES * 64) kq_rows(const RowsArgs a) {
    extern __shared__ __attribute__((aligned(16))) uint8_t smem[];
    if (RDIAG(a) & 256) return;
    const uint64_t st0 = RSTAMPS(a) ? __builtin_amdgcn_s_memrealtime() : 0;
    const int lane = threadIdx.x & 63;
    const int wave = __builtin_amdgcn_readfirstlane(threadIdx.x >> 6);
    const RowsLayout L = rows_layout(a.nb, TMASK, a.bR, a.rpw, __builtin_amdgcn_readfirstlane((int)(blockDim.x >> 6)));

    const int gw = wave * gridDim.x + blockIdx.x;
    WaveWork ww;
    int m = 0;
#pragma unroll
    for (int i = 1; i < MI355X_MAX_FUSED; ++i)
        if (i < a.n_desc && gw >= a.wave_prefix[i]) m = i;
    ww.m = m;
    const int j = gw - a.wave_prefix[m];
    const int base = a.rbase[m], rem = a.rrem[m];
    ww.r0 = j * base + (j < rem ? j : rem);
    ww.nrows = gw < a.waves_total ? base + (j < rem ? 1 : 0) : 0;

    if (TMASK == 1) {
        rows_body<Q4_K, FUSEDQ, PRO>(a, ww, smem, L, wave, lane, st0);
    } else if (TMASK == 2) {
        rows_body<Q5_K, FUSEDQ, PRO>(a, ww, smem, L, wave, lane, st0);
    } else if (TMASK == 4) {
        rows_body<Q6_K, FUSEDQ, PRO>(a, ww, smem, L, wave, lane, st0);
    } else {
        const int type = a.type[m];
        if (type == Q6_K) rows_body<Q6_K, FUSEDQ, PRO>(a, ww, smem, L, wave, lane, st0);
        else if (type == Q5_K) rows_body<Q5_K, FUSEDQ, PRO>(a, ww, smem, L, wave, lane, st0);
        else rows_body<Q4_K, FUSEDQ, PRO>(a, ww, smem, L, wave, lane, st0);
    }
}

#define KQ_ROWS_INST(TM, FQ, PR) template __global__ void kq_rows<TM, FQ, PR>(const RowsArgs a);
#define KQ_ROWS_INST_T(TM)        \
    KQ_ROWS_INST(TM, true, 0)     \
    KQ_ROWS_INST(TM, true, 1)     \
    KQ_ROWS_INST(TM, true, 2)     \
    KQ_ROWS_INST(TM, false, 0)
KQ_ROWS_INST_T(1)
KQ_ROWS_INST_T(2)
KQ_ROWS_INST_T(4)
KQ_ROWS_INST_T(7)

#ifndef KQ_ROWS_DYN_RR
#define KQ_ROWS_DYN_RR 0
#endif
namespace {
static_assert(MI355X_MAX_FUSED == 4, "four matrices at most");
struct DynUnit {
    const uint8_t *src;
    int rows, flat, G, T;
};
}

template <int TYPE, bool FUSEDQ, int PRO>
__device__ __forceinline__ void rows_dyn_body(const RowsArgs &a, uint8_t *smem, const RowsDynLayout &L, int wave,
                                              int lane, uint64_t st0) {
    uint64_t sx = 0, sq = 0, sf = 0;
    constexpr int BSZ = block_bytes(TYPE);
    constexpr int GRAN = rows_gran(TYPE);
    constexpr int NI = rows_ni(TYPE);
    constexpr int SLOT = rows_slot(TYPE);
    constexpr int D = rows_depth(TYPE);
    static_assert(D >= 2 && D <= 4, "vm_wait_k covers 3 steps in flight");
    const int nb = a.nb, U = a.dyn_u, P = a.dyn_p, bR = a.bR;
    const int nwv = __builtin_amdgcn_readfirstlane((int)(blockDim.x >> 6));
    const int b = (int)blockIdx.x;
    const int q = lane >> 2, s = lane & 3;
    uint8_t *const ring = smem + L.ring + wave * L.ring_stride;
    uint8_t *const ring_end = ring + D * SLOT;
    Rec *const recs = (Rec *)(smem + L.recs + wave * L.recs_stride);
    float *const outs = (float *)(smem + L.outs);
    uint32_t *const cnt = (uint32_t *)(smem + L.cnt);
    const uint8_t *const actq = smem + L.act;

    const int N = a.n_rows[0];
    const int ush = a.dyn_ush;
    const int rbase = a.rbase[0], rrem = a.rrem[0];
    const int r0 = b * rbase + (b < rrem ? b : rrem);
    const int nr = rbase + (b < rrem ? 1 : 0);
    const int nu = (nr + U - 1) >> ush;
    const int units = a.n_desc * nu, nflat = a.n_desc * nr;
    const int64_t rowb = (int64_t)nb * BSZ;
    auto row_of = [&](int f) { return r0 + f; };
    auto unit_of = [&](int u) {
        DynUnit d;
        const int m = (u >= nu ? 1 : 0) + (u >= 2 * nu ? 1 : 0) + (u >= 3 * nu ? 1 : 0);
        const int lr = (u - m * nu) << ush;
        d.rows = nr - lr < U ? nr - lr : U;
        d.flat = m * nr + lr;
        const uint8_t *w = m == 0 ? a.w[0] : m == 1 ? a.w[1] : m == 2 ? a.w[2] : a.w[3];
        d.src = w + (int64_t)(r0 + lr) * rowb;
        d.G = d.rows * nb;
        d.T = (d.G + ROWS_SB - 1) / ROWS_SB;
        return d;
    };
    const int nstat = nwv * P < units ? nwv * P : units;

    uint32_t ul = 0, uh = 0, ug = 0, uf = 0;
    int ki = -1, is = 0, iT = 0, issued = 0;
    bool idone = false, iwait = false;
    const uint8_t *is16 = nullptr, *il16 = nullptr;
    uint8_t *islot = ring;
    auto take = [&](int u) {
        ++ki;
        const DynUnit d = unit_of(u);
        const bool mine = lane == (ki & 7);
        ul = mine ? (uint32_t)(uintptr_t)d.src : ul;
        uh = mine ? (uint32_t)((uintptr_t)d.src >> 32) : uh;
        ug = mine ? (uint32_t)(d.G | (d.rows << 16)) : ug;
        uf = mine ? (uint32_t)d.flat : uf;
        is16 = (const uint8_t *)((uintptr_t)d.src & ~(uintptr_t)15);
        il16 = (const uint8_t *)((uintptr_t)(d.src + (int64_t)d.G * BSZ - 1) & ~(uintptr_t)15);
        iT = d.T;
        is = 0;
    };
    auto next_unit = [&](bool claim_ok) {
        const int k = ki + 1;
        if (k < P) {
            const int u = wave * P + k;
            if (u < nstat) take(u);
            else idone = true;
            return;
        }
        if (!claim_ok) {
            iwait = true;
            return;
        }
        iwait = false;
#if KQ_ROWS_DYN_RR
        const int uu = nwv * P + (k - P) * nwv + wave;
#else
        uint32_t u = 0;
        if (lane == 0) u = __hip_atomic_fetch_add(cnt, 1u, __ATOMIC_RELAXED, __HIP_MEMORY_SCOPE_WORKGROUP);
        const int uu = __builtin_amdgcn_readfirstlane((int)u);
#endif
        if (uu < units) take(uu);
        else idone = true;
    };
    auto issue = [&](bool claim_ok) {
        const uint8_t *base = is16 + (int64_t)is * (ROWS_SB * BSZ) + 16 * lane;
        if (is + 1 < iT) {
#pragma unroll
            for (int i = 0; i < NI; ++i)
                if (i + 1 < NI || lane < GRAN - 64 * (NI - 1)) dma16_nt(base + 1024 * i, (LDS void *)(islot + 1024 * i));
        } else {
#pragma unroll
            for (int i = 0; i < NI; ++i) {
                const uint8_t *p = base + 1024 * i;
                if (i + 1 < NI || lane < GRAN - 64 * (NI - 1))
                    dma16_nt(p < il16 ? p : il16, (LDS void *)(islot + 1024 * i));
            }
        }
        islot = islot + SLOT == ring_end ? ring : islot + SLOT;
        ++is;
        ++issued;
        if (is == iT) next_unit(claim_ok);
    };
    next_unit(false);

    const int f0 = 64 * wave + lane;
    const int fm = (f0 >= nr ? 1 : 0) + (f0 >= 2 * nr ? 1 : 0) + (f0 >= 3 * nr ? 1 : 0);
    const float *fres = fm == 0 ? a.res[0] : fm == 1 ? a.res[1] : fm == 2 ? a.res[2] : a.res[3];
    const int frow = row_of(f0 - fm * nr);
    uint32_t rv = 0;

    if (FUSEDQ) {
        const int PASS = 4 * nwv;
        u32x4 xv[ROWS_QPASS][4] = {};
        u32x4 x2v[ROWS_QPASS][4] = {};
        const int qiters = (nb + PASS - 1) / PASS;
        int qw = 0;
#pragma unroll
        for (int i = 0; i < ROWS_QPASS; ++i) qw += (i < qiters && PASS * i + 4 * wave < nb) ? 1 : 0;
#pragma unroll
        for (int i = 0; i < ROWS_QPASS; ++i) {
            if (i < qw) {
                const int j = PASS * i + 4 * wave + (lane >> 4);
                const int bb = j < nb ? j : nb - 1;
                const float *xp = a.x + (int64_t)bb * QK + 16 * (lane & 15);
#pragma unroll
                for (int k = 0; k < 4; ++k) xv[i][k] = gload16_asm(xp + 4 * k);
                if (PRO != ROWS_PRO_NONE) {
                    const float *x2p = a.x2 + (int64_t)bb * QK + 16 * (lane & 15);
#pragma unroll
                    for (int k = 0; k < 4; ++k) x2v[i][k] = gload16_asm(x2p + 4 * k);
                }
            }
        }
        rv = gload4_asm(fres && f0 < nflat && frow < N ? fres + frow : a.x);
        if (ki < 0) {
            const uint8_t *xb = (const uint8_t *)a.x + 16 * lane;
#pragma unroll
            for (int i = 0; i < NI; ++i)
                if (i + 1 == NI) dma16_nt_lanes(xb, (LDS void *)(islot + 1024 * i), lane, GRAN - 64 * (NI - 1));
                else dma16_nt(xb, (LDS void *)(islot + 1024 * i));
        } else {
            const uint8_t *base = is16 + 16 * lane;
            const uint8_t *lim = iT > 1 ? base + 1024 * (NI - 1) : base + 1024 * (NI - 1) < il16 ? base + 1024 * (NI - 1) : il16;
#pragma unroll
            for (int i = 0; i + 1 < NI; ++i) {
                const uint8_t *p = base + 1024 * i;
                dma16_nt(iT > 1 || p < il16 ? p : il16, (LDS void *)(islot + 1024 * i));
            }
            dma16_nt_lanes(lim, (LDS void *)(islot + 1024 * (NI - 1)), lane, GRAN - 64 * (NI - 1));
            islot = islot + SLOT == ring_end ? ring : islot + SLOT;
            ++is;
            ++issued;
            if (is == iT) next_unit(false);
        }
        vm_wait<NI + 1>();
        if (RSTAMPS(a)) sx = __builtin_amdgcn_s_memrealtime();
        asm volatile("" : "+v"(xv[0][0]), "+v"(xv[0][1]), "+v"(xv[0][2]), "+v"(xv[0][3]), "+v"(xv[1][0]),
                     "+v"(xv[1][1]), "+v"(xv[1][2]), "+v"(xv[1][3]), "+v"(xv[2][0]), "+v"(xv[2][1]),
                     "+v"(xv[2][2]), "+v"(xv[2][3]));
        if (PRO != ROWS_PRO_NONE) {
#pragma unroll
            for (int i = 0; i < ROWS_QPASS; ++i)
#pragma unroll
                for (int k = 0; k < 4; ++k) asm volatile("" : "+v"(x2v[i][k]));
        }
        if (PRO == ROWS_PRO_SWIGLU) {
#pragma unroll
            for (int i = 0; i < ROWS_QPASS; ++i)
                if (i < qw)
#pragma unroll
                    for (int k = 0; k < 4; ++k) xv[i][k] = swiglu4(xv[i][k], x2v[i][k]);
        } else if (PRO == ROWS_PRO_NORM) {
            double *sums = (double *)(smem + L.sums);
#pragma unroll
            for (int i = 0; i < ROWS_QPASS; ++i) {
                if (i < qw) {
                    const int j = PASS * i + 4 * wave + (lane >> 4);
                    double sq = 0.0;
                    if (j < nb) {
                        float v[16];
#pragma unroll
                        for (int k = 0; k < 4; ++k) {
                            v[4 * k] = __uint_as_float(xv[i][k].x), v[4 * k + 1] = __uint_as_float(xv[i][k].y);
                            v[4 * k + 2] = __uint_as_float(xv[i][k].z), v[4 * k + 3] = __uint_as_float(xv[i][k].w);
                        }
                        sq = sumsq16(v);
                    }
                    sq = row16_sum(sq);
                    if (j < nb && (lane & 15) == 0) sums[j] = sq;
                }
            }
            asm volatile("s_waitcnt lgkmcnt(0)\n\ts_barrier" ::: "memory");
            double tot = seq_sum_lanes(sums, nb, lane);
            if (rms_mean_ambiguous(div_by_count(tot, (int64_t)nb * QK), (int64_t)nb * QK))
                tot = seq_sumsq_wave(a.x, (int64_t)nb * QK, lane);
            const float mean = (float)div_by_count(tot, (int64_t)nb * QK);
            const float scale = 1.0f / sqrtf(mean + a.eps);
#pragma unroll
            for (int i = 0; i < ROWS_QPASS; ++i)
                if (i < qw)
#pragma unroll
                    for (int k = 0; k < 4; ++k) xv[i][k] = normmul4(xv[i][k], x2v[i][k], scale);
        }
#pragma unroll 1
        for (int i = 0; i < qw; ++i) {
            u32x4 cur[4];
#pragma unroll
            for (int k = 0; k < 4; ++k) cur[k] = i == 0 ? xv[0][k] : i == 1 ? xv[1][k] : xv[2][k];
            const int j = PASS * i + 4 * wave + (lane >> 4);
            if (j < nb) quant16_store(cur, lane & 15, smem + L.act + Q8L_STRIDE * j);
        }
        if (RSTAMPS(a)) {
            asm volatile("s_waitcnt lgkmcnt(0)" ::: "memory");
            sq = __builtin_amdgcn_s_memrealtime();
        }
    } else {
        const int ng = nb * (Q8L_STRIDE / 16);
        for (int j = wave; 64 * j < ng; j += nwv) {
            const int k = 64 * j + lane;
            if (k < ng) dma16(a.xq + 16 * k, (LDS void *)(smem + L.act + 1024 * j));
        }
        rv = gload4_asm(fres && f0 < nflat && frow < N ? fres + frow : (const float *)a.xq);
        if (!idone && !iwait && ki >= 0) issue(false);
        vm_wait_k<NI>(issued);
    }
    while (!idone && !iwait && ki >= 0 && issued < D) issue(false);
    if (wave == 0 && lane == 0) *cnt = (uint32_t)(nwv * P);
    asm volatile("s_waitcnt lgkmcnt(0)\n\ts_barrier" ::: "memory");
    if (iwait) next_unit(true);
    while (!idone && ki >= 0 && issued < D) issue(true);
    const uint64_t st1 = RSTAMPS(a) ? __builtin_amdgcn_s_memrealtime() : 0;

    int kc = 0, cs = 0, cT = 0, cG = 0, cmis = 0, crows = 0, io = 0, rr = 0;
    int bro = 0;
    uint32_t bfl = 0;
    auto consume_unit = [&](int k) {
        const uint32_t gr = (uint32_t)__builtin_amdgcn_readlane((int)ug, k & 7);
        const int flat = __builtin_amdgcn_readlane((int)uf, k & 7);
        cG = (int)(gr & 0xffffu);
        crows = (int)(gr >> 16);
        cT = (cG + ROWS_SB - 1) / ROWS_SB;
        cmis = (int)((uint32_t)__builtin_amdgcn_readlane((int)ul, k & 7) & 15u);
        bfl = lane >= bro && lane < bro + crows ? (uint32_t)(flat + lane - bro) : bfl;
        cs = 0;
        io = q;
        rr = bro;
        while (io >= nb) {
            io -= nb;
            ++rr;
        }
    };
    auto replay = [&]() {
        wave_lds_fence();
        if (lane < bro) {
            float v = 0.f;
            const Rec *rc = recs + lane;
#pragma unroll 4
            for (int i = 0; i < nb; ++i) v = chain_step(TYPE, rc[i * bR], v);
            outs[bfl] = v;
        }
        wave_lds_fence();
        bro = 0;
    };
    int consumed = 0;
    if (issued > 0) consume_unit(0);
    const uint8_t *cslot = ring;
#pragma unroll 1
    while (consumed < issued) {
        vm_wait_k<NI>(issued - consumed - 1);
        if (ROWS_SB * cs + q < cG) {
            const uint8_t *blk = cslot + cmis + q * BSZ;
            const uint8_t *ab = actq + io * Q8L_STRIDE;
            QuadOut r = TYPE == Q4_K ? quad_q4K(blk, ab, s) : TYPE == Q5_K ? quad_q5K(blk, ab, s) : quad_q6K(blk, ab, s);
            const int isum = quad_sum(r.isum);
            const int imin = quad_sum(r.imin);
            if (s == 0) {
                const float yd = *(const float *)ab;
                Rec rec;
                if (TYPE == Q6_K) {
                    rec.a = isum - 32 * imin;
                    rec.b = 0;
                    rec.c = h2f(r.dh) * yd;
                    rec.e = 0.f;
                } else {
                    rec.a = isum;
                    rec.b = imin;
                    rec.c = yd * h2f(r.dh & 0xffffu);
                    rec.e = yd * h2f(r.dh >> 16);
                }
                recs[io * bR + rr] = rec;
            }
        }
        cslot = cslot + SLOT == ring_end ? ring : cslot + SLOT;
        ++consumed;
        ++cs;
        if (!idone) issue(true);
        if (RSTAMPS(a) && consumed == 1) sf = __builtin_amdgcn_s_memrealtime();
        if (cs == cT) {
            bro += crows;
            if (bro + U > bR || consumed == issued) replay();
            ++kc;
            if (consumed < issued) consume_unit(kc);
        } else {
            io += ROWS_SB;
            while (io >= nb) {
                io -= nb;
                ++rr;
            }
        }
    }

    const uint64_t st2 = RSTAMPS(a) ? __builtin_amdgcn_s_memrealtime() : 0;
    asm volatile("s_waitcnt vmcnt(0)" ::: "memory");
    asm volatile("" : "+v"(rv));
    asm volatile("s_waitcnt lgkmcnt(0)\n\ts_barrier" ::: "memory");
    for (int f = f0; f < nflat; f += 64 * nwv) {
        const int m = (f >= nr ? 1 : 0) + (f >= 2 * nr ? 1 : 0) + (f >= 3 * nr ? 1 : 0);
        const int row = f == f0 ? frow : row_of(f - m * nr);
        if (row >= N) continue;
        const float *res = m == 0 ? a.res[0] : m == 1 ? a.res[1] : m == 2 ? a.res[2] : a.res[3];
        float *y = m == 0 ? a.y[0] : m == 1 ? a.y[1] : m == 2 ? a.y[2] : a.y[3];
        float v = outs[f];
        if (res) v = v + (f == f0 ? __uint_as_float(rv) : res[row]);
        store_y(y + row, v);
    }
    if (a.epi) {
        const int n4 = a.epi_n & ~3;
        for (int f = f0; f < nr; f += 64 * nwv) {
            const int r = row_of(f);
            if (r >= N) continue;
            const float gv = outs[f], uv = outs[nr + f];
            store_y(a.epi_y + r, r < n4 ? v_silu(gv) * uv : (gv / (1.0f + expf(-gv))) * uv);
        }
    }
    if (RSTAMPS(a)) {
        const int64_t o = ((int64_t)blockIdx.x * ROWS_WAVES + wave) * 8;
        if (lane == 0 && o + 7 < a.stamps_cap) {
            RSTAMPS(a)[o] = st0;
            RSTAMPS(a)[o + 1] = st1;
            RSTAMPS(a)[o + 2] = st2;
            RSTAMPS(a)[o + 3] = __builtin_amdgcn_s_memrealtime();
            RSTAMPS(a)[o + 4] = sx;
            RSTAMPS(a)[o + 5] = sq;
            RSTAMPS(a)[o + 6] = sf;
            RSTAMPS(a)[o + 7] = (uint64_t)(ki + 1);
        }
    }
}
template <int TMASK, bool FUSEDQ, int PRO>
__global__ void __launch_bounds__(ROWS_WAVES * 64) kq_rows_dyn(const RowsArgs a) {
    extern __shared__ __attribute__((aligned(16))) uint8_t smem[];
    const uint64_t st0 = RSTAMPS(a) ? __builtin_amdgcn_s_memrealtime() : 0;
    const int lane = threadIdx.x & 63;
    const int wave = __builtin_amdgcn_readfirstlane(threadIdx.x >> 6);
    const RowsDynLayout L =
        rows_dyn_layout(a.nb, TMASK, a.bR, a.rpw, __builtin_amdgcn_readfirstlane((int)(blockDim.x >> 6)));
    constexpr int TYPE = TMASK == 1 ? Q4_K : TMASK == 2 ? Q5_K : Q6_K;
    rows_dyn_body<TYPE, FUSEDQ, PRO>(a, smem, L, wave, lane, st0);
}

#define KQ_ROWS_DYN_INST(TM, FQ, PR) template __global__ void kq_rows_dyn<TM, FQ, PR>(const RowsArgs a);
#define KQ_ROWS_DYN_INST_T(TM)        \
    KQ_ROWS_DYN_INST(TM, true, 0)     \
    KQ_ROWS_DYN_INST(TM, true, 1)     \
    KQ_ROWS_DYN_INST(TM, true, 2)     \
    KQ_ROWS_DYN_INST(TM, false, 0)
KQ_ROWS_DYN_INST_T(1)
KQ_ROWS_DYN_INST_T(2)
KQ_ROWS_DYN_INST_T(4)

}
```

Before: 1328 tok/s.

## Hoist hot kernel arguments to leading scalars and batch-load kernarg struct

Row-GEMV and attention-decode kernels now receive the most-used fields (x, x2, w0, res0, nb, packed config) as leading scalar parameters. The rest of RowsArgs/AttnArgs, reordered so hot fields come first, is fetched with a few wide s_load_dwordx16/x8 instructions at entry instead of many scattered scalar loads. get_rows also stages the quantized row blocks in LDS with one coalesced 16-byte load per thread. The aim is to cut kernel-prologue latency on the many small decode kernels. The cost is hand-written kernarg offset assumptions that depend on struct layout, guarded by static_asserts, plus extra host-side validation.

```diff
diff --git a/ggml-neon-opt_amd/csrc/kq_api.hip b/ggml-neon-opt_amd/csrc/kq_api.hip
--- a/ggml-neon-opt_amd/csrc/kq_api.hip
+++ b/ggml-neon-opt_amd/csrc/kq_api.hip
@@ -19,9 +19,9 @@
 __global__ void kq_gemv(const GemvArgs a);
 __global__ void kq_quantize_q8K(const float *x, int64_t x_stride, uint8_t *y, int nb, int64_t nblocks);
 template <int TMASK, bool FUSEDQ, int PRO>
-__global__ void kq_rows(const RowsArgs a);
+__global__ void kq_rows(KQ_ROWS_PARAMS);
 template <int TMASK, bool FUSEDQ, int PRO>
-__global__ void kq_rows_dyn(const RowsArgs a);
+__global__ void kq_rows_dyn(KQ_ROWS_PARAMS);
 template <bool AM>
 __global__ void kq_quantize_q8L(const float *x, int64_t x_stride, uint8_t *y, int nb, int64_t nblocks);
 template <int TYPE, int RT, int CW>
@@ -528,12 +528,21 @@
     const RowsArgs &a = pl.a;
     if (a.waves_total == 0) return MI355X_OK;
     allow_lds((const void *)pl.fn, pl.lds);
+    const void *x = pl.fusedq ? (const void *)a.x : (const void *)a.xq;
+    const int pass = 4 * pl.nwv;
+    const int qiters = pl.fusedq ? (a.nb + pass - 1) / pass : 0;
+    if (pl.nwv < 1 || pl.nwv > ROWS_WAVES || qiters > ROWS_QPASS || a.n_desc < 1 || a.n_desc > MI355X_MAX_FUSED)
+        return MI355X_E_INVAL;
+    const int cfg = rows_cfg(pl.nwv, qiters, a.n_desc, a.diag & 0x1ff);
+    const int grid = (int)pl.grid.x;
     hipEvent_t e0, e1;
     if (timing_slot(stream, e0, e1)) {
-        hipExtLaunchKernelGGL(pl.fn, pl.grid, dim3(pl.nwv * 64), (uint32_t)pl.lds, stream, e0, e1, 0, a);
+        hipExtLaunchKernelGGL(pl.fn, pl.grid, dim3(pl.nwv * 64), (uint32_t)pl.lds, stream, e0, e1, 0, x, a.x2, a.w[0],
+                              a.res[0], a.nb, a.waves_total, grid, cfg, a.rbase[0], a.rrem[0], a);
         timing_log(rows_name(pl), rows_bytes(a, pl.fusedq), e0, e1);
     } else {
-        hipLaunchKernelGGL(pl.fn, pl.grid, dim3(pl.nwv * 64), pl.lds, stream, a);
+        hipLaunchKernelGGL(pl.fn, pl.grid, dim3(pl.nwv * 64), pl.lds, stream, x, a.x2, a.w[0], a.res[0], a.nb,
+                           a.waves_total, grid, cfg, a.rbase[0], a.rrem[0], a);
     }
     const hipError_t e = hipGetLastError();
     return e == hipSuccess ? MI355X_OK : (int)e;
diff --git a/ggml-neon-opt_amd/csrc/kq_common.h b/ggml-neon-opt_amd/csrc/kq_common.h
--- a/ggml-neon-opt_amd/csrc/kq_common.h
+++ b/ggml-neon-opt_amd/csrc/kq_common.h
@@ -81,35 +81,43 @@
 #endif
 constexpr int ROWS_PF = KQ_ROWS_PF;
 
+#define KQ_ROWS_PARAMS                                                                                        \
+    const void *x, const float *x2, const uint8_t *w0, const float *res0, int nb, int waves_total, int grid, \
+        int cfg, int rbase0, int rrem0, const RowsArgs a
+__host__ __device__ constexpr int rows_cfg(int nwv, int qiters, int n_desc, int diag) {
+    return nwv | (qiters << 8) | (n_desc << 12) | (diag << 16);
+}
+
 struct RowsArgs {
-    int n_desc;
-    int nb;
+    int bR;
     int rpw;
-    int waves_total;
-    int pre0;
-    int pf;
-    int bR;
-    int xmode;
-    int diag;
     int wave_prefix[MI355X_MAX_FUSED + 1];
+    int epi;
     int rbase[MI355X_MAX_FUSED];
     int rrem[MI355X_MAX_FUSED];
     int type[MI355X_MAX_FUSED];
     const uint8_t *w[MI355X_MAX_FUSED];
+    const float *res[MI355X_MAX_FUSED];
     float *y[MI355X_MAX_FUSED];
+    float *epi_y;
+    float eps;
+    int epi_n, epi_wave_off;
+    int dyn_u, dyn_p, dyn_ush;
+    int n_rows[MI355X_MAX_FUSED];
+    uint64_t *stamps;
+    int64_t stamps_cap;
+    int n_desc;
+    int nb;
+    int waves_total;
     const float *x;
     const uint8_t *xq;
-    uint64_t *stamps;
-    int64_t stamps_cap;
+    const float *x2;
     int pro;
-    float eps;
-    const float *x2;
-    const float *res[MI355X_MAX_FUSED];
-    int n_rows[MI355X_MAX_FUSED];
-    int epi, epi_n, epi_wave_off;
-    float *epi_y;
+    int diag;
+    int pre0;
+    int pf;
+    int xmode;
     int64_t prio_bytes;
-    int dyn_u, dyn_p, dyn_ush;
 };
 constexpr int ROWS_PRO_NONE = 0, ROWS_PRO_NORM = 1, ROWS_PRO_SWIGLU = 2;
 constexpr int ROWS_X_ROT = 1, ROWS_X_BAR = 2, ROWS_X_PIPE = 4;
diff --git a/ggml-neon-opt_amd/csrc/kq_internal.h b/ggml-neon-opt_amd/csrc/kq_internal.h
--- a/ggml-neon-opt_amd/csrc/kq_internal.h
+++ b/ggml-neon-opt_amd/csrc/kq_internal.h
@@ -23,7 +23,7 @@
 int plan_gemv(const mi355x_gemv_desc *d, int n_desc, int64_t K, int64_t M, int ncol, bool fusedq, bool debug,
               GemvPlan &pl);
 int launch_gemv(const GemvPlan &pl, hipStream_t stream);
-typedef void (*rows_fn)(const RowsArgs);
+typedef void (*rows_fn)(KQ_ROWS_PARAMS);
 struct RowsPlan {
     RowsArgs a;
     dim3 grid;
diff --git a/ggml-neon-opt_amd/csrc/kq_ops.hip b/ggml-neon-opt_amd/csrc/kq_ops.hip
--- a/ggml-neon-opt_amd/csrc/kq_ops.hip
+++ b/ggml-neon-opt_amd/csrc/kq_ops.hip
@@ -25,27 +25,45 @@
 
 namespace kq {
 
+constexpr int GETROWS_STAGE = ((15 + 8 * 210 + 15) / 16) * 16;
 __global__ void __launch_bounds__(256) kq_get_rows(int type, const uint8_t *__restrict__ table, int64_t k,
                                                    int64_t row_stride, int64_t n_rows,
                                                    const int32_t *__restrict__ ids, float *__restrict__ out) {
+    __shared__ __attribute__((aligned(16))) uint8_t stage[GETROWS_STAGE];
     const int64_t r = blockIdx.y;
     const int64_t e0 = ((int64_t)blockIdx.x * 256 + threadIdx.x) * 8;
-    if (e0 >= k) return;
+    const bool live = e0 < k;
     const int64_t id = ids[r];
     float *y = out + r * k + e0;
     if (id < 0 || id >= n_rows) {
-#pragma unroll
-        for (int i = 0; i < 8; ++i) y[i] = __builtin_nanf("");
+        if (live) {
+#pragma unroll
+            for (int i = 0; i < 8; ++i) y[i] = __builtin_nanf("");
+        }
         return;
     }
-    const uint8_t *row = table + id * row_stride;
+    const uint8_t *grow = table + id * row_stride;
     if (type == MI355X_TYPE_F32) {
-        const float *s = (const float *)row + e0;
-#pragma unroll
-        for (int i = 0; i < 8; ++i) y[i] = s[i];
+        if (live) {
+            const float *s = (const float *)grow + e0;
+#pragma unroll
+            for (int i = 0; i < 8; ++i) y[i] = s[i];
+        }
         return;
     }
-    const int64_t b = e0 / QK;
+    const int bsz = block_bytes(type);
+    const int64_t b0 = (int64_t)blockIdx.x * 8;
+    const int64_t left = k / QK - b0;
+    const int nblk = (int)(left < 8 ? left : 8);
+    const uint8_t *src = grow + b0 * bsz;
+    const uint32_t mis = (uint32_t)((uintptr_t)src & 15u);
+    const int ng = (int)((mis + (uint32_t)(nblk * bsz) + 15u) / 16u);
+    if ((int)threadIdx.x < ng)
+        *(u32x4 *)(stage + 16 * threadIdx.x) = *(const u32x4 *)(src - mis + 16 * threadIdx.x);
+    __syncthreads();
+    if (!live) return;
+    const uint8_t *row = stage + mis;
+    const int64_t b = e0 / QK - b0;
     const int e = (int)(e0 % QK);
     if (type == MI355X_TYPE_Q4_K || type == MI355X_TYPE_Q5_K) {
         const bool q5 = type == MI355X_TYPE_Q5_K;
@@ -178,9 +196,44 @@
 #ifndef KQ_ATTN_KDMA1
 #define KQ_ATTN_KDMA1 0
 #endif
+#define KQ_ATTN_PARAMS                                                                                      \
+    const float *q, const float *k, const float *v, const int32_t *pos, const float *rope_table, uint16_t *k_cache, \
+        uint16_t *v_cache, const AttnArgs a0
+constexpr int kAttnArgsOff = 14 * 4;
+static_assert(offsetof(AttnArgs, out) == 56 && offsetof(AttnArgs, rope_row) == 88 && offsetof(AttnArgs, v_lds) == 104 &&
+                  sizeof(AttnArgs) == 112 && alignof(AttnArgs) == 8,
+              "attn_entry reads out .. n_tok as 8 + 4 + 2 dwords");
+typedef uint32_t u32x2s __attribute__((ext_vector_type(2)));
+typedef uint32_t u32x4s __attribute__((ext_vector_type(4)));
+typedef uint32_t u32x8s __attribute__((ext_vector_type(8)));
+__device__ __forceinline__ AttnArgs attn_entry(const float *q, const float *k, const float *v, const int32_t *pos,
+                                               const float *rope_table, uint16_t *k_cache, uint16_t *v_cache) {
+    const auto *ka = __builtin_amdgcn_kernarg_segment_ptr();
+    u32x8s r0;
+    u32x4s r1;
+    u32x2s r2;
+    asm volatile("s_load_dwordx8 %0, %3, %4\n\t"
+                 "s_load_dwordx4 %1, %3, %5\n\t"
+                 "s_load_dwordx2 %2, %3, %6\n\t"
+                 "s_waitcnt lgkmcnt(0)"
+                 : "=&s"(r0), "=&s"(r1), "=&s"(r2)
+                 : "s"(ka), "i"(kAttnArgsOff + 56), "i"(kAttnArgsOff + 88), "i"(kAttnArgsOff + 104));
+    AttnArgs a;
+    a.q = q, a.k = k, a.v = v, a.pos = pos, a.rope_table = rope_table, a.k_cache = k_cache, a.v_cache = v_cache;
+    a.out = (float *)(uintptr_t)((uint64_t)r0[0] | ((uint64_t)r0[1] << 32));
+    a.n_ctx = (int)r0[2], a.n_head = (int)r0[3], a.n_head_kv = (int)r0[4], a.head_dim = (int)r0[5];
+    a.scale = __uint_as_float(r0[6]);
+    a.diag = (int)r0[7];
+    a.rope_row = (int)r1[0], a.no_store = (int)r1[1];
+    a.q8_out = (uint8_t *)(uintptr_t)((uint64_t)r1[2] | ((uint64_t)r1[3] << 32));
+    a.v_lds = (int)r2[0], a.n_tok = (int)r2[1];
+    return a;
+}
+
 template <int HD, bool BATCH, int DS = 1, int TPH = 256, bool KD1 = false>
-__global__ void __launch_bounds__(TPH) kq_attn_decode(const AttnArgs a) {
+__global__ void __launch_bounds__(TPH) kq_attn_decode(KQ_ATTN_PARAMS) {
     extern __shared__ __attribute__((aligned(16))) uint8_t smem[];
+    const AttnArgs a = attn_entry(q, k, v, pos, rope_table, k_cache, v_cache);
     int h = blockIdx.x / DS, ds = blockIdx.x % DS;
     if ((a.n_head & 7) == 0) {
         const int x = blockIdx.x & 7, i = blockIdx.x >> 3;
@@ -1007,6 +1060,7 @@
                             glds, s, a);
     }
     AttnArgs b = a;
+#define KQ_ATTN_LEAD(b) (b).q, (b).k, (b).v, (b).pos, (b).rope_table, (b).k_cache, (b).v_cache, (b)
     const int ds = attn_slices(a);
     if (path == MI355X_ATTN_PATH_SPLIT4 || path == MI355X_ATTN_PATH_SPLIT8) {
         const size_t lds = attn_lds_v(a.head_dim, a.n_ctx, ds);
@@ -1015,7 +1069,7 @@
     if (a.head_dim == HD && ds == DS) {                                                                    \
         allow_lds((const void *)kq_attn_decode<HD, true, DS>, lds);                                        \
         return timed_launch("kq::kq_attn_decode<" #HD ", true, " #DS ">", bytes, kq_attn_decode<HD, true, DS>, \
-                            grid, dim3(256), lds, s, b);                                                   \
+                            grid, dim3(256), lds, s, KQ_ATTN_LEAD(b));                                                   \
     }
         KQ_ATTN_SPLIT_LAUNCH(64, 4)
         KQ_ATTN_SPLIT_LAUNCH(64, 8)
@@ -1035,11 +1089,11 @@
         if (a.head_dim == 64) {
             allow_lds((const void *)kq_attn_decode<64, true, 1, 256, true>, lds);
             return timed_launch("kq::kq_attn_decode<64, true, 1, kd1>", bytes, kq_attn_decode<64, true, 1, 256, true>,
-                                dim3(a.n_head), dim3(256), lds, s, b);
+                                dim3(a.n_head), dim3(256), lds, s, KQ_ATTN_LEAD(b));
         }
         allow_lds((const void *)kq_attn_decode<128, true, 1, 256, true>, lds);
         return timed_launch("kq::kq_attn_decode<128, true, 1, kd1>", bytes, kq_attn_decode<128, true, 1, 256, true>,
-                            dim3(a.n_head), dim3(256), lds, s, b);
+                            dim3(a.n_head), dim3(256), lds, s, KQ_ATTN_LEAD(b));
     }
     b.v_lds = a.n_ctx > KQ_ATTN_BATCH_CTX && a.n_ctx % 8 == 0 && attn_lds_v(a.head_dim, a.n_ctx) <= 160 * 1024 &&
               ((uintptr_t)a.v_cache & 15u) == 0 && KQ_ATTN_VLDS;
@@ -1048,14 +1102,16 @@
     if (a.head_dim == 64) {
         if (!batch)
             return timed_launch("kq::kq_attn_decode<64, false>", bytes, kq_attn_decode<64, false, 1, KQ_ATTN_TPH64>,
-                                dim3(a.n_head), dim3(KQ_ATTN_TPH64), lds, s, b);
+                                dim3(a.n_head), dim3(KQ_ATTN_TPH64), lds, s, KQ_ATTN_LEAD(b));
         if (b.v_lds) allow_lds((const void *)kq_attn_decode<64, true>, lds);
-        return timed_launch("kq::kq_attn_decode<64, true>", bytes, kq_attn_decode<64, true>, dim3(a.n_head), dim3(256), lds, s, b);
-    }
-    if (!batch) return timed_launch("kq::kq_attn_decode<128, false>", bytes, kq_attn_decode<128, false>, dim3(a.n_head), dim3(256), lds, s, b);
+        return timed_launch("kq::kq_attn_decode<64, true>", bytes, kq_attn_decode<64, true>, dim3(a.n_head), dim3(256), lds, s, KQ_ATTN_LEAD(b));
+    }
+    if (!batch) return timed_launch("kq::kq_attn_decode<128, false>", bytes, kq_attn_decode<128, false>, dim3(a.n_head), dim3(256), lds, s, KQ_ATTN_LEAD(b));
     if (b.v_lds) allow_lds((const void *)kq_attn_decode<128, true>, lds);
-    return timed_launch("kq::kq_attn_decode<128, true>", bytes, kq_attn_decode<128, true>, dim3(a.n_head), dim3(256), lds, s, b);
-}
+    return timed_launch("kq::kq_attn_decode<128, true>", bytes, kq_attn_decode<128, true>, dim3(a.n_head), dim3(256), lds, s, KQ_ATTN_LEAD(b));
+}
+
+#undef KQ_ATTN_LEAD
 
 std::atomic<int> g_prompt_impl{MI355X_ATTN_GROUP};
 
diff --git a/ggml-neon-opt_amd/csrc/kq_rows.hip b/ggml-neon-opt_amd/csrc/kq_rows.hip
--- a/ggml-neon-opt_amd/csrc/kq_rows.hip
+++ b/ggml-neon-opt_amd/csrc/kq_rows.hip
@@ -8,11 +8,13 @@
 #define KQ_ROWS_DIAG 0
 #endif
 #if KQ_ROWS_DIAG
-#define RDIAG(a) ((a).diag)
-#define RSTAMPS(a) ((a).stamps)
+#define RDIAG(ld) ((ld).diag)
+#define RSTAMPS(h) ((h).stamps)
+#define RSTAMP() __builtin_amdgcn_s_memrealtime()
 #else
-#define RDIAG(a) 0
-#define RSTAMPS(a) ((uint64_t *)nullptr)
+#define RDIAG(ld) 0
+#define RSTAMPS(h) ((uint64_t *)nullptr)
+#define RSTAMP() ((uint64_t)0)
 #endif
 
 #ifndef KQ_ROWS_XMODE
@@ -167,27 +169,190 @@
     return e == hipSuccess ? MI355X_OK : (int)e;
 }
 
-template <int TYPE, bool FUSEDQ, int PRO>
-__device__ __forceinline__ void rows_body(const RowsArgs &a, const WaveWork &ww, uint8_t *smem, const RowsLayout &L,
-                                          int wave, int lane, uint64_t st0) {
+struct RowsLead {
+    const void *x;
+    const float *x2;
+    const uint8_t *w0;
+    const float *res0;
+    int nb, waves_total, grid, nwv, qiters, n_desc, diag, rbase0, rrem0;
+};
+__device__ __forceinline__ RowsLead rows_lead(const void *x, const float *x2, const uint8_t *w0, const float *res0,
+                                              int nb, int waves_total, int grid, int cfg, int rbase0, int rrem0) {
+    RowsLead ld;
+    ld.x = x, ld.x2 = x2, ld.w0 = w0, ld.res0 = res0;
+    ld.nb = nb, ld.waves_total = waves_total, ld.grid = grid;
+    ld.nwv = cfg & 0xff, ld.qiters = (cfg >> 8) & 0xf, ld.n_desc = (cfg >> 12) & 0xf, ld.diag = (cfg >> 16) & 0x1ff;
+    ld.rbase0 = rbase0, ld.rrem0 = rrem0;
+    return ld;
+}
+
+typedef uint32_t u32x8s __attribute__((ext_vector_type(8)));
+typedef uint32_t u32x16s __attribute__((ext_vector_type(16)));
+constexpr int kRowsArgsOff = 14 * 4;
+static_assert(alignof(RowsArgs) == 8 && kRowsArgsOff % 8 == 0, "RowsArgs follows the leading parameters unpadded");
+#define RA_DW(f) ((int)(offsetof(RowsArgs, f) / 4))
+#if KQ_ROWS_DIAG
+typedef u32x16s rows_run_tail;
+#define KQ_ROWS_RUN_TAIL "s_load_dwordx16"
+static_assert(offsetof(RowsArgs, stamps_cap) + 8 <= 64 * 4 && sizeof(RowsArgs) >= 64 * 4, "entry run: 64 dwords");
+#else
+typedef u32x8s rows_run_tail;
+#define KQ_ROWS_RUN_TAIL "s_load_dwordx8"
+static_assert(offsetof(RowsArgs, n_rows) + 16 <= 56 * 4 && sizeof(RowsArgs) >= 56 * 4, "entry run: 56 dwords");
+#endif
+struct RowsRun {
+    u32x16s a, b, c;
+    rows_run_tail d;
+    template <int I>
+    __device__ __forceinline__ uint32_t dw() const {
+        if constexpr (I < 16) return a[I];
+        else if constexpr (I < 32) return b[I - 16];
+        else if constexpr (I < 48) return c[I - 32];
+        else return d[I - 48];
+    }
+    template <int I>
+    __device__ __forceinline__ int i32() const {
+        return (int)dw<I>();
+    }
+    template <class T, int I>
+    __device__ __forceinline__ T *ptr() const {
+        return (T *)(uintptr_t)((uint64_t)dw<I>() | ((uint64_t)dw<I + 1>() << 32));
+    }
+};
+__device__ __forceinline__ RowsRun rows_fetch() {
+    const auto *ka = __builtin_amdgcn_kernarg_segment_ptr();
+    RowsRun r;
+    asm volatile("s_load_dwordx16 %0, %4, %5\n\t"
+                 "s_load_dwordx16 %1, %4, %6\n\t"
+                 "s_load_dwordx16 %2, %4, %7\n\t" KQ_ROWS_RUN_TAIL " %3, %4, %8\n\t"
+                 "s_waitcnt lgkmcnt(0)"
+                 : "=&s"(r.a), "=&s"(r.b), "=&s"(r.c), "=&s"(r.d)
+                 : "s"(ka), "i"(kRowsArgsOff), "i"(kRowsArgsOff + 64), "i"(kRowsArgsOff + 128), "i"(kRowsArgsOff + 192));
+    return r;
+}
+
+template <class T>
+__device__ __forceinline__ T sreg(T v) {
+    asm volatile("" : "+s"(v));
+    return v;
+}
+
+struct RowsHot {
+    int m, r0, nrows;
+    int type, bR, rpw;
+    const uint8_t *w;
+    const float *res;
+    float *y;
+    float eps;
+    int epi, epi_n, epi_wave_off;
+    float *epi_y;
+    uint64_t *stamps;
+    int64_t stamps_cap;
+};
+
+template <int TMASK>
+__device__ __forceinline__ RowsHot rows_resolve(const RowsLead &ld, int gw) {
+    const RowsRun r = rows_fetch();
+    RowsHot h;
+    h.bR = r.i32<RA_DW(bR)>(), h.rpw = r.i32<RA_DW(rpw)>();
+    h.epi = r.i32<RA_DW(epi)>(), h.epi_n = r.i32<RA_DW(epi_n)>(), h.epi_wave_off = r.i32<RA_DW(epi_wave_off)>();
+    h.eps = __uint_as_float(r.dw<RA_DW(eps)>());
+    h.epi_y = r.ptr<float, RA_DW(epi_y)>();
+#if KQ_ROWS_DIAG
+    h.stamps = r.ptr<uint64_t, RA_DW(stamps)>();
+    h.stamps_cap = (int64_t)(uintptr_t)r.ptr<uint8_t, RA_DW(stamps_cap)>();
+#else
+    h.stamps = nullptr, h.stamps_cap = 0;
+#endif
+    h.m = 0, h.w = ld.w0, h.res = ld.res0;
+    h.type = TMASK == 7 ? sreg(r.i32<RA_DW(type)>()) : 0;
+    h.y = sreg(r.ptr<float, RA_DW(y)>());
+    int j = gw, base = ld.rbase0, rem = ld.rrem0;
+    if (ld.n_desc > 1) {
+        const int p1 = sreg(r.i32<RA_DW(wave_prefix) + 1>()), p2 = sreg(r.i32<RA_DW(wave_prefix) + 2>()),
+                  p3 = sreg(r.i32<RA_DW(wave_prefix) + 3>());
+        const int b1 = sreg(r.i32<RA_DW(rbase) + 1>()), b2 = sreg(r.i32<RA_DW(rbase) + 2>()), b3 = sreg(r.i32<RA_DW(rbase) + 3>());
+        const int e1 = sreg(r.i32<RA_DW(rrem) + 1>()), e2 = sreg(r.i32<RA_DW(rrem) + 2>()), e3 = sreg(r.i32<RA_DW(rrem) + 3>());
+        const uint8_t *w1 = sreg(r.ptr<const uint8_t, RA_DW(w) + 2>()), *w2 = sreg(r.ptr<const uint8_t, RA_DW(w) + 4>()),
+                      *w3 = sreg(r.ptr<const uint8_t, RA_DW(w) + 6>());
+        const float *s1 = sreg(r.ptr<const float, RA_DW(res) + 2>()), *s2 = sreg(r.ptr<const float, RA_DW(res) + 4>()),
+                    *s3 = sreg(r.ptr<const float, RA_DW(res) + 6>());
+        float *y1 = sreg(r.ptr<float, RA_DW(y) + 2>()), *y2 = sreg(r.ptr<float, RA_DW(y) + 4>()), *y3 = sreg(r.ptr<float, RA_DW(y) + 6>());
+        int m = gw >= p1 ? 1 : 0;
+        if (ld.n_desc > 2 && gw >= p2) m = 2;
+        if (ld.n_desc > 3 && gw >= p3) m = 3;
+        h.m = m;
+        j = gw - (m == 0 ? 0 : m == 1 ? p1 : m == 2 ? p2 : p3);
+        base = m == 0 ? base : m == 1 ? b1 : m == 2 ? b2 : b3;
+        rem = m == 0 ? rem : m == 1 ? e1 : m == 2 ? e2 : e3;
+        if (TMASK == 7) {
+            const int t1 = sreg(r.i32<RA_DW(type) + 1>()), t2 = sreg(r.i32<RA_DW(type) + 2>()), t3 = sreg(r.i32<RA_DW(type) + 3>());
+            h.type = m == 0 ? h.type : m == 1 ? t1 : m == 2 ? t2 : t3;
+        }
+        h.w = m == 0 ? h.w : m == 1 ? w1 : m == 2 ? w2 : w3;
+        h.res = m == 0 ? h.res : m == 1 ? s1 : m == 2 ? s2 : s3;
+        h.y = m == 0 ? h.y : m == 1 ? y1 : m == 2 ? y2 : y3;
+    }
+    h.r0 = j * base + (j < rem ? j : rem);
+    h.nrows = gw < ld.waves_total ? base + (j < rem ? 1 : 0) : 0;
+    return h;
+}
+
+template <int TYPE, bool FUSEDQ, int PRO, int TMASK, class Resolve>
+__device__ __forceinline__ void rows_body(const RowsArgs &a, const RowsLead &ld, uint8_t *smem, int wave, int lane,
+                                          uint64_t st0, Resolve resolve) {
     constexpr int BSZ = block_bytes(TYPE);
     constexpr int GRAN = rows_gran(TYPE);
     constexpr int NI = rows_ni(TYPE);
     constexpr int SLOT = rows_slot(TYPE);
     constexpr int D = rows_depth(TYPE);
     static_assert(D >= 2 && D <= 4, "vm_wait_k covers 3 steps in flight");
-    const int nb = a.nb, bR = a.bR;
-    const int nwv = __builtin_amdgcn_readfirstlane((int)(blockDim.x >> 6));
+    const int nb = ld.nb;
+    const int nwv = ld.nwv;
     const int q = lane >> 2, s = lane & 3;
+
+    const int PASS = 4 * nwv;
+    const int xm = !FUSEDQ ? 0 : KQ_ROWS_XMODE >= 0 ? KQ_ROWS_XMODE : a.xmode;
+    u32x4 xv[ROWS_QPASS][4] = {};
+    u32x4 x2v[ROWS_QPASS][4] = {};
+    int qw = 0;
+    const int rot = (xm & ROWS_X_ROT) ? (int)(blockIdx.x % (unsigned)nb) : 0;
+    auto sbk = [&](int j) {
+        int b = (j < nb ? j : nb - 1) + rot;
+        return b >= nb ? b - nb : b;
+    };
+    if (FUSEDQ) {
+        const float *const x = (const float *)ld.x;
+#pragma unroll
+        for (int i = 0; i < ROWS_QPASS; ++i) qw += (i < ld.qiters && PASS * i + 4 * wave < nb) ? 1 : 0;
+#pragma unroll
+        for (int i = 0; i < ROWS_QPASS; ++i) {
+            if (i < qw) {
+                const int b = sbk(PASS * i + 4 * wave + (lane >> 4));
+                const float *xp = x + (int64_t)b * QK + 16 * (lane & 15);
+#pragma unroll
+                for (int k = 0; k < 4; ++k) xv[i][k] = gload16_asm(xp + 4 * k);
+                if (PRO != ROWS_PRO_NONE) {
+                    const float *x2p = ((RDIAG(ld) & 16) ? x : ld.x2) + (int64_t)b * QK + 16 * (lane & 15);
+#pragma unroll
+                    for (int k = 0; k < 4; ++k) x2v[i][k] = gload16_asm(x2p + 4 * k);
+                }
+            }
+        }
+    }
+    const RowsHot h = resolve();
+    const uint64_t sa = RSTAMP();
+    const int bR = h.bR;
+    const RowsLayout L = rows_layout(nb, TMASK, bR, h.rpw, nwv);
     uint8_t *const ring = smem + L.ring + wave * L.ring_stride;
     uint8_t *const ring_end = ring + D * SLOT;
     Rec *const recs = (Rec *)(smem + L.recs + wave * L.recs_stride);
     float *const outs = (float *)(smem + L.outs + wave * L.outs_stride);
     const uint8_t *const actq = smem + L.act;
 
-    const int G = ww.nrows * nb;
+    const int G = h.nrows * nb;
     const int T = (G + ROWS_SB - 1) / ROWS_SB;
-    const uint8_t *src = a.w[ww.m] + (int64_t)ww.r0 * nb * BSZ;
+    const uint8_t *src = h.w + (int64_t)h.r0 * nb * BSZ;
     const uint32_t mis = (uint32_t)((uintptr_t)src & 15u);
     const uint8_t *s16 = src - mis;
     const uint8_t *last16 =
@@ -215,7 +380,7 @@
         ++it_;
     };
 
-    const float *const res_p = a.res[ww.m];
+    const float *const res_p = h.res;
     uint32_t rv = 0;
 
     const int pre_req = KQ_ROWS_PRE0 < 0 ? a.pre0 : KQ_ROWS_PRE0;
@@ -223,40 +388,14 @@
     const int pre0 = T >= pre_cap ? pre_cap : (T > 0 ? T : 0);
     uint64_t sx = 0, sq = 0, sf = 0;
     if (FUSEDQ) {
-        const int PASS = 4 * nwv;
-        const int xm = KQ_ROWS_XMODE >= 0 ? KQ_ROWS_XMODE : a.xmode;
-        u32x4 xv[ROWS_QPASS][4] = {};
-        u32x4 x2v[ROWS_QPASS][4] = {};
-        const int qiters = (nb + PASS - 1) / PASS;
-        int qw = 0;
-#pragma unroll
-        for (int i = 0; i < ROWS_QPASS; ++i) qw += (i < qiters && PASS * i + 4 * wave < nb) ? 1 : 0;
-        const int rot = (xm & ROWS_X_ROT) ? (int)(blockIdx.x % (unsigned)nb) : 0;
-        auto sbk = [&](int j) {
-            int b = (j < nb ? j : nb - 1) + rot;
-            return b >= nb ? b - nb : b;
-        };
+        const float *const x = (const float *)ld.x;
         constexpr int pro = PRO;
         constexpr int PL = PRO != ROWS_PRO_NONE ? 8 : 4;
-#pragma unroll
-        for (int i = 0; i < ROWS_QPASS; ++i) {
-            if (i < qw) {
-                const int b = sbk(PASS * i + 4 * wave + (lane >> 4));
-                const float *xp = a.x + (int64_t)b * QK + 16 * (lane & 15);
-#pragma unroll
-                for (int k = 0; k < 4; ++k) xv[i][k] = gload16_asm(xp + 4 * k);
-                if (PRO != ROWS_PRO_NONE) {
-                    const float *x2p = ((RDIAG(a) & 16) ? a.x : a.x2) + (int64_t)b * QK + 16 * (lane & 15);
-#pragma unroll
-                    for (int k = 0; k < 4; ++k) x2v[i][k] = gload16_asm(x2p + 4 * k);
-                }
-            }
-        }
-        rv = gload4_asm(res_p && ww.nrows > 0 ? res_p + ww.r0 + (lane < ww.nrows ? lane : 0) : a.x);
+        rv = gload4_asm(res_p && h.nrows > 0 ? res_p + h.r0 + (lane < h.nrows ? lane : 0) : x);
         if (xm & ROWS_X_BAR) asm volatile("s_barrier" ::: "memory");
         constexpr bool kConstPre = KQ_ROWS_PRE0 == 1 && KQ_ROWS_L2PF == 0;
         if (kConstPre && T == 0) {
-            const uint8_t *xb = (const uint8_t *)a.x + 16 * lane;
+            const uint8_t *xb = (const uint8_t *)x + 16 * lane;
 #pragma unroll
             for (int i = 0; i < NI; ++i)
                 if (KQ_ROWS_MASKED && i + 1 == NI) dma16_nt_lanes(xb, (LDS void *)(islot + 1024 * i), lane, GRAN - 64 * (NI - 1));
@@ -299,15 +438,15 @@
                 if (i < qw) {
                     vm_wait_dyn((qw - 1 - i) * PL + tail);
                     pin();
-                    if (pro == ROWS_PRO_SWIGLU && !(RDIAG(a) & 32)) {
+                    if (pro == ROWS_PRO_SWIGLU && !(RDIAG(ld) & 32)) {
 #pragma unroll
                         for (int k = 0; k < 4; ++k) xv[i][k] = swiglu4(xv[i][k], x2v[i][k]);
                     }
                     const int j = PASS * i + 4 * wave + (lane >> 4);
-                    if (j < nb && !(RDIAG(a) & 64)) quant16_store(xv[i], lane & 15, smem + L.act + Q8L_STRIDE * sbk(j));
+                    if (j < nb && !(RDIAG(ld) & 64)) quant16_store(xv[i], lane & 15, smem + L.act + Q8L_STRIDE * sbk(j));
                 }
             }
-            if (RSTAMPS(a)) sx = sq = __builtin_amdgcn_s_memrealtime();
+            if (RSTAMPS(h)) sx = sq = __builtin_amdgcn_s_memrealtime();
         } else {
             if (KQ_ROWS_LINT_BREAK) {
             } else if (kConstPre && KQ_ROWS_MASKED == 2) {
@@ -318,7 +457,7 @@
                 vm_wait_dyn(tail);
             }
             pin();
-            if (RDIAG(a) & 32) {
+            if (RDIAG(ld) & 32) {
             } else if (pro == ROWS_PRO_SWIGLU) {
 #pragma unroll
                 for (int i = 0; i < ROWS_QPASS; ++i)
@@ -348,25 +487,25 @@
                 asm volatile("s_waitcnt lgkmcnt(0)\n\ts_barrier" ::: "memory");
                 double tot = seq_sum_lanes(sums, nb, lane);
                 if (rms_mean_ambiguous(div_by_count(tot, (int64_t)nb * QK), (int64_t)nb * QK))
-                    tot = seq_sumsq_wave(a.x, (int64_t)nb * QK, lane);
+                    tot = seq_sumsq_wave(x, (int64_t)nb * QK, lane);
                 const float mean = (float)div_by_count(tot, (int64_t)nb * QK);
-                const float scale = 1.0f / sqrtf(mean + a.eps);
+                const float scale = 1.0f / sqrtf(mean + h.eps);
 #pragma unroll
                 for (int i = 0; i < ROWS_QPASS; ++i)
                     if (i < qw)
 #pragma unroll
                         for (int k = 0; k < 4; ++k) xv[i][k] = normmul4(xv[i][k], x2v[i][k], scale);
             }
-            if (RSTAMPS(a)) sx = __builtin_amdgcn_s_memrealtime();
+            if (RSTAMPS(h)) sx = __builtin_amdgcn_s_memrealtime();
 #pragma unroll 1
             for (int i = 0; i < qw; ++i) {
                 u32x4 cur[4];
 #pragma unroll
                 for (int k = 0; k < 4; ++k) cur[k] = i == 0 ? xv[0][k] : i == 1 ? xv[1][k] : xv[2][k];
                 const int j = PASS * i + 4 * wave + (lane >> 4);
-                if (j < nb && !(RDIAG(a) & 64)) quant16_store(cur, lane & 15, smem + L.act + Q8L_STRIDE * sbk(j));
-            }
-            if (RSTAMPS(a)) {
+                if (j < nb && !(RDIAG(ld) & 64)) quant16_store(cur, lane & 15, smem + L.act + Q8L_STRIDE * sbk(j));
+            }
+            if (RSTAMPS(h)) {
                 asm volatile("s_waitcnt lgkmcnt(0)" ::: "memory");
                 sq = __builtin_amdgcn_s_memrealtime();
             }
@@ -375,14 +514,14 @@
         const int ng = nb * (Q8L_STRIDE / 16);
         for (int j = wave; 64 * j < ng; j += nwv) {
             const int k = 64 * j + lane;
-            if (k < ng) dma16(a.xq + 16 * k, (LDS void *)(smem + L.act + 1024 * j));
+            if (k < ng) dma16((const uint8_t *)ld.x + 16 * k, (LDS void *)(smem + L.act + 1024 * j));
         }
         for (int j = 0; j < pre0; ++j) issue();
         vm_wait_k<NI>(pre0);
     }
     while (it_ < D && it_ < T) issue();
     asm volatile("s_waitcnt lgkmcnt(0)\n\ts_barrier" ::: "memory");
-    const uint64_t st1 = RSTAMPS(a) ? __builtin_amdgcn_s_memrealtime() : 0;
+    const uint64_t st1 = RSTAMPS(h) ? __builtin_amdgcn_s_memrealtime() : 0;
 
     int io = q, rr = 0;
     while (io >= nb) {
@@ -415,7 +554,7 @@
         } else {
             vm_wait_k<NI>(T - t - 1);
         }
-        if (!(RDIAG(a) & 8) && ROWS_SB * t + q < G) {
+        if (!(RDIAG(ld) & 8) && ROWS_SB * t + q < G) {
             const uint8_t *blk = cslot + mis + q * BSZ;
             const uint8_t *ab = actq + io * Q8L_STRIDE;
             QuadOut r = TYPE == Q4_K ? quad_q4K(blk, ab, s) : TYPE == Q5_K ? quad_q5K(blk, ab, s) : quad_q6K(blk, ab, s);
@@ -452,10 +591,10 @@
             }
         }
         if (it_ < T) issue();
-        if (RSTAMPS(a) && t == 0) sf = __builtin_amdgcn_s_memrealtime();
+        if (RSTAMPS(h) && t == 0) sf = __builtin_amdgcn_s_memrealtime();
         if (ROWS_SB * (t + 1) >= bend) {
             wave_lds_fence();
-            const int nr = bR < ww.nrows - brow ? bR : ww.nrows - brow;
+            const int nr = bR < h.nrows - brow ? bR : h.nrows - brow;
             if (lane < nr) {
                 float v = 0.f;
                 const Rec *rc = recs + lane;
@@ -470,88 +609,80 @@
         }
     }
     if (KQ_ROWS_PRIO) __builtin_amdgcn_s_setprio(0);
-    const uint64_t st2 = RSTAMPS(a) ? __builtin_amdgcn_s_memrealtime() : 0;
+    const uint64_t st2 = RSTAMPS(h) ? __builtin_amdgcn_s_memrealtime() : 0;
     if (pf_on) {
         asm volatile("" ::"v"(pf_sink));
     }
 
-    if (ww.nrows > 0) {
+    if (h.nrows > 0) {
         wave_lds_fence();
-        float *y = a.y[ww.m] + ww.r0;
+        float *y = h.y + h.r0;
         if (res_p) {
             asm volatile("s_waitcnt vmcnt(0)" ::: "memory");
             asm volatile("" : "+v"(rv));
-            for (int k = 0; k < ww.nrows; k += 64)
-                if (k + lane < ww.nrows)
-                    store_y(y + k + lane, outs[k + lane] + (k == 0 ? __uint_as_float(rv) : res_p[ww.r0 + k + lane]));
+            for (int k = 0; k < h.nrows; k += 64)
+                if (k + lane < h.nrows)
+                    store_y(y + k + lane, outs[k + lane] + (k == 0 ? __uint_as_float(rv) : res_p[h.r0 + k + lane]));
         } else {
-            for (int k = 0; k < ww.nrows; k += 64)
-                if (k + lane < ww.nrows) store_y(y + k + lane, outs[k + lane]);
-        }
-    }
-    if (a.epi && !(RDIAG(a) & 128)) {
+            for (int k = 0; k < h.nrows; k += 64)
+                if (k + lane < h.nrows) store_y(y + k + lane, outs[k + lane]);
+        }
+    }
+    if (h.epi && !(RDIAG(ld) & 128)) {
         asm volatile("s_waitcnt lgkmcnt(0)\n\ts_barrier" ::: "memory");
-        if (ww.m == 1 && ww.nrows > 0) {
-            const float *gouts = (const float *)(smem + L.outs + (wave - a.epi_wave_off) * L.outs_stride);
-            const int n4 = a.epi_n & ~3;
-            for (int k = 0; k < ww.nrows; k += 64)
-                if (k + lane < ww.nrows) {
-                    const int r = ww.r0 + k + lane;
+        if (h.m == 1 && h.nrows > 0) {
+            const float *gouts = (const float *)(smem + L.outs + (wave - h.epi_wave_off) * L.outs_stride);
+            const int n4 = h.epi_n & ~3;
+            for (int k = 0; k < h.nrows; k += 64)
+                if (k + lane < h.nrows) {
+                    const int r = h.r0 + k + lane;
                     const float gv = gouts[k + lane], uv = outs[k + lane];
-                    store_y(a.epi_y + r, r < n4 ? v_silu(gv) * uv : (gv / (1.0f + expf(-gv))) * uv);
+                    store_y(h.epi_y + r, r < n4 ? v_silu(gv) * uv : (gv / (1.0f + expf(-gv))) * uv);
                 }
         }
     }
-    if (RSTAMPS(a)) {
+    if (RSTAMPS(h)) {
         const int64_t o = ((int64_t)blockIdx.x * ROWS_WAVES + wave) * 8;
-        if (lane == 0 && o + 7 < a.stamps_cap) {
-            RSTAMPS(a)[o] = st0;
-            RSTAMPS(a)[o + 1] = st1;
-            RSTAMPS(a)[o + 2] = st2;
-            RSTAMPS(a)[o + 3] = __builtin_amdgcn_s_memrealtime();
-            RSTAMPS(a)[o + 4] = sx;
-            RSTAMPS(a)[o + 5] = sq;
-            RSTAMPS(a)[o + 6] = sf;
+        if (lane == 0 && o + 7 < h.stamps_cap) {
+            RSTAMPS(h)[o] = st0;
+            RSTAMPS(h)[o + 1] = st1;
+            RSTAMPS(h)[o + 2] = st2;
+            RSTAMPS(h)[o + 3] = __builtin_amdgcn_s_memrealtime();
+            RSTAMPS(h)[o + 4] = sx;
+            RSTAMPS(h)[o + 5] = sq;
+            RSTAMPS(h)[o + 6] = sf;
+            RSTAMPS(h)[o + 7] = sa;
         }
     }
 }
 
 template <int TMASK, bool FUSEDQ, int PRO>
-__global__ void __launch_bounds__(ROWS_WAVES * 64) kq_rows(const RowsArgs a) {
+__global__ void __launch_bounds__(ROWS_WAVES * 64) kq_rows(KQ_ROWS_PARAMS) {
     extern __shared__ __attribute__((aligned(16))) uint8_t smem[];
-    if (RDIAG(a) & 256) return;
-    const uint64_t st0 = RSTAMPS(a) ? __builtin_amdgcn_s_memrealtime() : 0;
+    const RowsLead ld = rows_lead(x, x2, w0, res0, nb, waves_total, grid, cfg, rbase0, rrem0);
+    if (RDIAG(ld) & 256) return;
+    const uint64_t st0 = RSTAMP();
     const int lane = threadIdx.x & 63;
     const int wave = __builtin_amdgcn_readfirstlane(threadIdx.x >> 6);
-    const RowsLayout L = rows_layout(a.nb, TMASK, a.bR, a.rpw, __builtin_amdgcn_readfirstlane((int)(blockDim.x >> 6)));
-
-    const int gw = wave * gridDim.x + blockIdx.x;
-    WaveWork ww;
-    int m = 0;
-#pragma unroll
-    for (int i = 1; i < MI355X_MAX_FUSED; ++i)
-        if (i < a.n_desc && gw >= a.wave_prefix[i]) m = i;
-    ww.m = m;
-    const int j = gw - a.wave_prefix[m];
-    const int base = a.rbase[m], rem = a.rrem[m];
-    ww.r0 = j * base + (j < rem ? j : rem);
-    ww.nrows = gw < a.waves_total ? base + (j < rem ? 1 : 0) : 0;
+    const int gw = wave * ld.grid + blockIdx.x;
+    auto resolve = [&]() { return rows_resolve<TMASK>(ld, gw); };
 
     if (TMASK == 1) {
-        rows_body<Q4_K, FUSEDQ, PRO>(a, ww, smem, L, wave, lane, st0);
+        rows_body<Q4_K, FUSEDQ, PRO, TMASK>(a, ld, smem, wave, lane, st0, resolve);
     } else if (TMASK == 2) {
-        rows_body<Q5_K, FUSEDQ, PRO>(a, ww, smem, L, wave, lane, st0);
+        rows_body<Q5_K, FUSEDQ, PRO, TMASK>(a, ld, smem, wave, lane, st0, resolve);
     } else if (TMASK == 4) {
-        rows_body<Q6_K, FUSEDQ, PRO>(a, ww, smem, L, wave, lane, st0);
+        rows_body<Q6_K, FUSEDQ, PRO, TMASK>(a, ld, smem, wave, lane, st0, resolve);
     } else {
-        const int type = a.type[m];
-        if (type == Q6_K) rows_body<Q6_K, FUSEDQ, PRO>(a, ww, smem, L, wave, lane, st0);
-        else if (type == Q5_K) rows_body<Q5_K, FUSEDQ, PRO>(a, ww, smem, L, wave, lane, st0);
-        else rows_body<Q4_K, FUSEDQ, PRO>(a, ww, smem, L, wave, lane, st0);
-    }
-}
-
-#define KQ_ROWS_INST(TM, FQ, PR) template __global__ void kq_rows<TM, FQ, PR>(const RowsArgs a);
+        const RowsHot h = resolve();
+        auto resolved = [&]() { return h; };
+        if (h.type == Q6_K) rows_body<Q6_K, FUSEDQ, PRO, TMASK>(a, ld, smem, wave, lane, st0, resolved);
+        else if (h.type == Q5_K) rows_body<Q5_K, FUSEDQ, PRO, TMASK>(a, ld, smem, wave, lane, st0, resolved);
+        else rows_body<Q4_K, FUSEDQ, PRO, TMASK>(a, ld, smem, wave, lane, st0, resolved);
+    }
+}
+
+#define KQ_ROWS_INST(TM, FQ, PR) template __global__ void kq_rows<TM, FQ, PR>(KQ_ROWS_PARAMS);
 #define KQ_ROWS_INST_T(TM)        \
     KQ_ROWS_INST(TM, true, 0)     \
     KQ_ROWS_INST(TM, true, 1)     \
@@ -573,9 +704,41 @@
 };
 }
 
-template <int TYPE, bool FUSEDQ, int PRO>
-__device__ __forceinline__ void rows_dyn_body(const RowsArgs &a, uint8_t *smem, const RowsDynLayout &L, int wave,
-                                              int lane, uint64_t st0) {
+struct RowsDynHot {
+    int bR, rpw, U, P, ush, N, epi, epi_n;
+    const uint8_t *w1, *w2, *w3;
+    const float *s1, *s2, *s3;
+    float *y0, *y1, *y2, *y3, *epi_y;
+    float eps;
+    uint64_t *stamps;
+    int64_t stamps_cap;
+};
+__device__ __forceinline__ RowsDynHot rows_dyn_resolve() {
+    const RowsRun r = rows_fetch();
+    RowsDynHot h;
+    h.bR = r.i32<RA_DW(bR)>(), h.rpw = r.i32<RA_DW(rpw)>();
+    h.U = r.i32<RA_DW(dyn_u)>(), h.P = r.i32<RA_DW(dyn_p)>(), h.ush = r.i32<RA_DW(dyn_ush)>(), h.N = r.i32<RA_DW(n_rows)>();
+    h.epi = r.i32<RA_DW(epi)>(), h.epi_n = r.i32<RA_DW(epi_n)>();
+    h.epi_y = r.ptr<float, RA_DW(epi_y)>();
+    h.eps = __uint_as_float(r.dw<RA_DW(eps)>());
+    h.w1 = sreg(r.ptr<const uint8_t, RA_DW(w) + 2>()), h.w2 = sreg(r.ptr<const uint8_t, RA_DW(w) + 4>());
+    h.w3 = sreg(r.ptr<const uint8_t, RA_DW(w) + 6>());
+    h.s1 = sreg(r.ptr<const float, RA_DW(res) + 2>()), h.s2 = sreg(r.ptr<const float, RA_DW(res) + 4>());
+    h.s3 = sreg(r.ptr<const float, RA_DW(res) + 6>());
+    h.y0 = sreg(r.ptr<float, RA_DW(y)>()), h.y1 = sreg(r.ptr<float, RA_DW(y) + 2>());
+    h.y2 = sreg(r.ptr<float, RA_DW(y) + 4>()), h.y3 = sreg(r.ptr<float, RA_DW(y) + 6>());
+#if KQ_ROWS_DIAG
+    h.stamps = r.ptr<uint64_t, RA_DW(stamps)>();
+    h.stamps_cap = (int64_t)(uintptr_t)r.ptr<uint8_t, RA_DW(stamps_cap)>();
+#else
+    h.stamps = nullptr, h.stamps_cap = 0;
+#endif
+    return h;
+}
+
+template <int TYPE, bool FUSEDQ, int PRO, int TMASK>
+__device__ __forceinline__ void rows_dyn_body(const RowsArgs &a, const RowsLead &ld, uint8_t *smem, int wave, int lane,
+                                              uint64_t st0) {
     uint64_t sx = 0, sq = 0, sf = 0;
     constexpr int BSZ = block_bytes(TYPE);
     constexpr int GRAN = rows_gran(TYPE);
@@ -583,10 +746,41 @@
     constexpr int SLOT = rows_slot(TYPE);
     constexpr int D = rows_depth(TYPE);
     static_assert(D >= 2 && D <= 4, "vm_wait_k covers 3 steps in flight");
-    const int nb = a.nb, U = a.dyn_u, P = a.dyn_p, bR = a.bR;
-    const int nwv = __builtin_amdgcn_readfirstlane((int)(blockDim.x >> 6));
+    const int nb = ld.nb;
+    const int nwv = ld.nwv;
     const int b = (int)blockIdx.x;
     const int q = lane >> 2, s = lane & 3;
+
+    const float *const x = (const float *)ld.x;
+    const int PASS = 4 * nwv;
+    u32x4 xv[ROWS_QPASS][4] = {};
+    u32x4 x2v[ROWS_QPASS][4] = {};
+    int qw = 0;
+    if (FUSEDQ) {
+#pragma unroll
+        for (int i = 0; i < ROWS_QPASS; ++i) qw += (i < ld.qiters && PASS * i + 4 * wave < nb) ? 1 : 0;
+#pragma unroll
+        for (int i = 0; i < ROWS_QPASS; ++i) {
+            if (i < qw) {
+                const int j = PASS * i + 4 * wave + (lane >> 4);
+                const int bb = j < nb ? j : nb - 1;
+                const float *xp = x + (int64_t)bb * QK + 16 * (lane & 15);
+#pragma unroll
+                for (int k = 0; k < 4; ++k) xv[i][k] = gload16_asm(xp + 4 * k);
+                if (PRO != ROWS_PRO_NONE) {
+                    const float *x2p = ld.x2 + (int64_t)bb * QK + 16 * (lane & 15);
+#pragma unroll
+                    for (int k = 0; k < 4; ++k) x2v[i][k] = gload16_asm(x2p + 4 * k);
+                }
+            }
+        }
+    }
+    const RowsDynHot h = rows_dyn_resolve();
+    const uint8_t *const w0 = ld.w0, *const w1 = h.w1, *const w2 = h.w2, *const w3 = h.w3;
+    const float *const s0 = ld.res0, *const s1 = h.s1, *const s2 = h.s2, *const s3 = h.s3;
+    float *const y0 = h.y0, *const y1 = h.y1, *const y2 = h.y2, *const y3 = h.y3;
+    const int U = h.U, P = h.P, bR = h.bR;
+    const RowsDynLayout L = rows_dyn_layout(nb, TMASK, bR, h.rpw, nwv);
     uint8_t *const ring = smem + L.ring + wave * L.ring_stride;
     uint8_t *const ring_end = ring + D * SLOT;
     Rec *const recs = (Rec *)(smem + L.recs + wave * L.recs_stride);
@@ -594,13 +788,13 @@
     uint32_t *const cnt = (uint32_t *)(smem + L.cnt);
     const uint8_t *const actq = smem + L.act;
 
-    const int N = a.n_rows[0];
-    const int ush = a.dyn_ush;
-    const int rbase = a.rbase[0], rrem = a.rrem[0];
+    const int N = h.N;
+    const int ush = h.ush;
+    const int rbase = ld.rbase0, rrem = ld.rrem0;
     const int r0 = b * rbase + (b < rrem ? b : rrem);
     const int nr = rbase + (b < rrem ? 1 : 0);
     const int nu = (nr + U - 1) >> ush;
-    const int units = a.n_desc * nu, nflat = a.n_desc * nr;
+    const int units = ld.n_desc * nu, nflat = ld.n_desc * nr;
     const int64_t rowb = (int64_t)nb * BSZ;
     auto row_of = [&](int f) { return r0 + f; };
     auto unit_of = [&](int u) {
@@ -609,7 +803,7 @@
         const int lr = (u - m * nu) << ush;
         d.rows = nr - lr < U ? nr - lr : U;
         d.flat = m * nr + lr;
-        const uint8_t *w = m == 0 ? a.w[0] : m == 1 ? a.w[1] : m == 2 ? a.w[2] : a.w[3];
+        const uint8_t *w = m == 0 ? w0 : m == 1 ? w1 : m == 2 ? w2 : w3;
         d.src = w + (int64_t)(r0 + lr) * rowb;
         d.G = d.rows * nb;
         d.T = (d.G + ROWS_SB - 1) / ROWS_SB;
@@ -681,36 +875,14 @@
 
     const int f0 = 64 * wave + lane;
     const int fm = (f0 >= nr ? 1 : 0) + (f0 >= 2 * nr ? 1 : 0) + (f0 >= 3 * nr ? 1 : 0);
-    const float *fres = fm == 0 ? a.res[0] : fm == 1 ? a.res[1] : fm == 2 ? a.res[2] : a.res[3];
+    const float *fres = fm == 0 ? s0 : fm == 1 ? s1 : fm == 2 ? s2 : s3;
     const int frow = row_of(f0 - fm * nr);
     uint32_t rv = 0;
 
     if (FUSEDQ) {
-        const int PASS = 4 * nwv;
-        u32x4 xv[ROWS_QPASS][4] = {};
-        u32x4 x2v[ROWS_QPASS][4] = {};
-        const int qiters = (nb + PASS - 1) / PASS;
-        int qw = 0;
-#pragma unroll
-        for (int i = 0; i < ROWS_QPASS; ++i) qw += (i < qiters && PASS * i + 4 * wave < nb) ? 1 : 0;
-#pragma unroll
-        for (int i = 0; i < ROWS_QPASS; ++i) {
-            if (i < qw) {
-                const int j = PASS * i + 4 * wave + (lane >> 4);
-                const int bb = j < nb ? j : nb - 1;
-                const float *xp = a.x + (int64_t)bb * QK + 16 * (lane & 15);
-#pragma unroll
-                for (int k = 0; k < 4; ++k) xv[i][k] = gload16_asm(xp + 4 * k);
-                if (PRO != ROWS_PRO_NONE) {
-                    const float *x2p = a.x2 + (int64_t)bb * QK + 16 * (lane & 15);
-#pragma unroll
-                    for (int k = 0; k < 4; ++k) x2v[i][k] = gload16_asm(x2p + 4 * k);
-                }
-            }
-        }
-        rv = gload4_asm(fres && f0 < nflat && frow < N ? fres + frow : a.x);
+        rv = gload4_asm(fres && f0 < nflat && frow < N ? fres + frow : x);
         if (ki < 0) {
-            const uint8_t *xb = (const uint8_t *)a.x + 16 * lane;
+            const uint8_t *xb = (const uint8_t *)x + 16 * lane;
 #pragma unroll
             for (int i = 0; i < NI; ++i)
                 if (i + 1 == NI) dma16_nt_lanes(xb, (LDS void *)(islot + 1024 * i), lane, GRAN - 64 * (NI - 1));
@@ -730,7 +902,7 @@
             if (is == iT) next_unit(false);
         }
         vm_wait<NI + 1>();
-        if (RSTAMPS(a)) sx = __builtin_amdgcn_s_memrealtime();
+        if (RSTAMPS(h)) sx = __builtin_amdgcn_s_memrealtime();
         asm volatile("" : "+v"(xv[0][0]), "+v"(xv[0][1]), "+v"(xv[0][2]), "+v"(xv[0][3]), "+v"(xv[1][0]),
                      "+v"(xv[1][1]), "+v"(xv[1][2]), "+v"(xv[1][3]), "+v"(xv[2][0]), "+v"(xv[2][1]),
                      "+v"(xv[2][2]), "+v"(xv[2][3]));
@@ -769,9 +941,9 @@
             asm volatile("s_waitcnt lgkmcnt(0)\n\ts_barrier" ::: "memory");
             double tot = seq_sum_lanes(sums, nb, lane);
             if (rms_mean_ambiguous(div_by_count(tot, (int64_t)nb * QK), (int64_t)nb * QK))
-                tot = seq_sumsq_wave(a.x, (int64_t)nb * QK, lane);
+                tot = seq_sumsq_wave(x, (int64_t)nb * QK, lane);
             const float mean = (float)div_by_count(tot, (int64_t)nb * QK);
-            const float scale = 1.0f / sqrtf(mean + a.eps);
+            const float scale = 1.0f / sqrtf(mean + h.eps);
 #pragma unroll
             for (int i = 0; i < ROWS_QPASS; ++i)
                 if (i < qw)
@@ -786,7 +958,7 @@
             const int j = PASS * i + 4 * wave + (lane >> 4);
             if (j < nb) quant16_store(cur, lane & 15, smem + L.act + Q8L_STRIDE * j);
         }
-        if (RSTAMPS(a)) {
+        if (RSTAMPS(h)) {
             asm volatile("s_waitcnt lgkmcnt(0)" ::: "memory");
             sq = __builtin_amdgcn_s_memrealtime();
         }
@@ -794,9 +966,9 @@
         const int ng = nb * (Q8L_STRIDE / 16);
         for (int j = wave; 64 * j < ng; j += nwv) {
             const int k = 64 * j + lane;
-            if (k < ng) dma16(a.xq + 16 * k, (LDS void *)(smem + L.act + 1024 * j));
-        }
-        rv = gload4_asm(fres && f0 < nflat && frow < N ? fres + frow : (const float *)a.xq);
+            if (k < ng) dma16((const uint8_t *)ld.x + 16 * k, (LDS void *)(smem + L.act + 1024 * j));
+        }
+        rv = gload4_asm(fres && f0 < nflat && frow < N ? fres + frow : (const float *)ld.x);
         if (!idone && !iwait && ki >= 0) issue(false);
         vm_wait_k<NI>(issued);
     }
@@ -805,7 +977,7 @@
     asm volatile("s_waitcnt lgkmcnt(0)\n\ts_barrier" ::: "memory");
     if (iwait) next_unit(true);
     while (!idone && ki >= 0 && issued < D) issue(true);
-    const uint64_t st1 = RSTAMPS(a) ? __builtin_amdgcn_s_memrealtime() : 0;
+    const uint64_t st1 = RSTAMPS(h) ? __builtin_amdgcn_s_memrealtime() : 0;
 
     int kc = 0, cs = 0, cT = 0, cG = 0, cmis = 0, crows = 0, io = 0, rr = 0;
     int bro = 0;
@@ -871,7 +1043,7 @@
         ++consumed;
         ++cs;
         if (!idone) issue(true);
-        if (RSTAMPS(a) && consumed == 1) sf = __builtin_amdgcn_s_memrealtime();
+        if (RSTAMPS(h) && consumed == 1) sf = __builtin_amdgcn_s_memrealtime();
         if (cs == cT) {
             bro += crows;
             if (bro + U > bR || consumed == issued) replay();
@@ -886,7 +1058,7 @@
         }
     }
 
-    const uint64_t st2 = RSTAMPS(a) ? __builtin_amdgcn_s_memrealtime() : 0;
+    const uint64_t st2 = RSTAMPS(h) ? __builtin_amdgcn_s_memrealtime() : 0;
     asm volatile("s_waitcnt vmcnt(0)" ::: "memory");
     asm volatile("" : "+v"(rv));
     asm volatile("s_waitcnt lgkmcnt(0)\n\ts_barrier" ::: "memory");
@@ -894,48 +1066,47 @@
         const int m = (f >= nr ? 1 : 0) + (f >= 2 * nr ? 1 : 0) + (f >= 3 * nr ? 1 : 0);
         const int row = f == f0 ? frow : row_of(f - m * nr);
         if (row >= N) continue;
-        const float *res = m == 0 ? a.res[0] : m == 1 ? a.res[1] : m == 2 ? a.res[2] : a.res[3];
-        float *y = m == 0 ? a.y[0] : m == 1 ? a.y[1] : m == 2 ? a.y[2] : a.y[3];
+        const float *res = m == 0 ? s0 : m == 1 ? s1 : m == 2 ? s2 : s3;
+        float *y = m == 0 ? y0 : m == 1 ? y1 : m == 2 ? y2 : y3;
         float v = outs[f];
         if (res) v = v + (f == f0 ? __uint_as_float(rv) : res[row]);
         store_y(y + row, v);
     }
-    if (a.epi) {
-        const int n4 = a.epi_n & ~3;
+    if (h.epi) {
+        const int n4 = h.epi_n & ~3;
         for (int f = f0; f < nr; f += 64 * nwv) {
             const int r = row_of(f);
             if (r >= N) continue;
             const float gv = outs[f], uv = outs[nr + f];
-            store_y(a.epi_y + r, r < n4 ? v_silu(gv) * uv : (gv / (1.0f + expf(-gv))) * uv);
-        }
-    }
-    if (RSTAMPS(a)) {
+            store_y(h.epi_y + r, r < n4 ? v_silu(gv) * uv : (gv / (1.0f + expf(-gv))) * uv);
+        }
+    }
+    if (RSTAMPS(h)) {
         const int64_t o = ((int64_t)blockIdx.x * ROWS_WAVES + wave) * 8;
-        if (lane == 0 && o + 7 < a.stamps_cap) {
-            RSTAMPS(a)[o] = st0;
-            RSTAMPS(a)[o + 1] = st1;
-            RSTAMPS(a)[o + 2] = st2;
-            RSTAMPS(a)[o + 3] = __builtin_amdgcn_s_memrealtime();
-            RSTAMPS(a)[o + 4] = sx;
-            RSTAMPS(a)[o + 5] = sq;
-            RSTAMPS(a)[o + 6] = sf;
-            RSTAMPS(a)[o + 7] = (uint64_t)(ki + 1);
+        if (lane == 0 && o + 7 < h.stamps_cap) {
+            RSTAMPS(h)[o] = st0;
+            RSTAMPS(h)[o + 1] = st1;
+            RSTAMPS(h)[o + 2] = st2;
+            RSTAMPS(h)[o + 3] = __builtin_amdgcn_s_memrealtime();
+            RSTAMPS(h)[o + 4] = sx;
+            RSTAMPS(h)[o + 5] = sq;
+            RSTAMPS(h)[o + 6] = sf;
+            RSTAMPS(h)[o + 7] = (uint64_t)(ki + 1);
         }
     }
 }
 template <int TMASK, bool FUSEDQ, int PRO>
-__global__ void __launch_bounds__(ROWS_WAVES * 64) kq_rows_dyn(const RowsArgs a) {
+__global__ void __launch_bounds__(ROWS_WAVES * 64) kq_rows_dyn(KQ_ROWS_PARAMS) {
     extern __shared__ __attribute__((aligned(16))) uint8_t smem[];
-    const uint64_t st0 = RSTAMPS(a) ? __builtin_amdgcn_s_memrealtime() : 0;
+    const RowsLead ld = rows_lead(x, x2, w0, res0, nb, waves_total, grid, cfg, rbase0, rrem0);
+    const uint64_t st0 = RSTAMP();
     const int lane = threadIdx.x & 63;
     const int wave = __builtin_amdgcn_readfirstlane(threadIdx.x >> 6);
-    const RowsDynLayout L =
-        rows_dyn_layout(a.nb, TMASK, a.bR, a.rpw, __builtin_amdgcn_readfirstlane((int)(blockDim.x >> 6)));
     constexpr int TYPE = TMASK == 1 ? Q4_K : TMASK == 2 ? Q5_K : Q6_K;
-    rows_dyn_body<TYPE, FUSEDQ, PRO>(a, smem, L, wave, lane, st0);
-}
-
-#define KQ_ROWS_DYN_INST(TM, FQ, PR) template __global__ void kq_rows_dyn<TM, FQ, PR>(const RowsArgs a);
+    rows_dyn_body<TYPE, FUSEDQ, PRO, TMASK>(a, ld, smem, wave, lane, st0);
+}
+
+#define KQ_ROWS_DYN_INST(TM, FQ, PR) template __global__ void kq_rows_dyn<TM, FQ, PR>(KQ_ROWS_PARAMS);
 #define KQ_ROWS_DYN_INST_T(TM)        \
     KQ_ROWS_DYN_INST(TM, true, 0)     \
     KQ_ROWS_DYN_INST(TM, true, 1)     \
```

After: 1383 tok/s, median of 6. 1.04x the previous value.
